# DearCaat/MHIM-MIL

Measured on AMD Instinct MI355X. Metric: patch-instances/sec through MHIM fwd+bwd, N=10k D=1024, higher is better.
Workload: dtype f32; 1 GPU; c2: MHIM(ABMIL) train step, one bag N=10000 D=1024 per GPU per step (teacher fwd + select + student fwd + bwd + Adam + EMA); rotating_bags_per_gpu=8, matrix_core_form=bf16x3, parallelism=dp1, launch=hipGraph replay, one graph per resident bag

## Files before the change

include/mhimx.h:

```cpp
#ifndef MHIMX_H
#define MHIMX_H

#include <stdint.h>

#ifdef __cplusplus
extern "C" {
#endif

#define MHIMX_VERSION 620

enum { MHIMX_ACT_NONE = 0, MHIMX_ACT_RELU = 1, MHIMX_ACT_GELU = 2, MHIMX_ACT_TANH = 3 };

enum { MHIMX_PREC_F32 = 0, MHIMX_PREC_F16S = 1, MHIMX_PREC_BF16X3 = 2 };

const char* mhimx_last_error(void);
int mhimx_version(void);


typedef struct {
  const float* A; int64_t lda; const int64_t* rows;
  const float* B; int64_t ldb;
  float* C; int64_t ldc;
  int64_t M, N, K;
  const float* bias;
// ... 257 lines not shown
  mhimx_reduce_list* defer;
} mhimx_merge_grad;
int64_t mhimx_merge_part_floats(void);
int mhimx_merge_fwd_part(void* stream, const mhimx_merge* m, const float* X, int64_t R, float* part, void* ws, int64_t ws_bytes);
int mhimx_merge_fwd_finish(void* stream, const mhimx_merge* m, const float* parts, int32_t W, int64_t R, float* z, float* q_new,
                           int32_t update_q, void* ws, int64_t ws_bytes);
int mhimx_merge_bwd(void* stream, const mhimx_merge* m, const float* X, int64_t R, const float* dz, float* dX,
                    const mhimx_merge_grad* g, void* ws, int64_t ws_bytes);
int mhimx_merge_bwd_park(const mhimx_merge* m, const float* X, int64_t R, const float* dz, float* dX, const mhimx_merge_grad* g, void* ws,
                         int64_t ws_bytes);

int mhimx_act_bwd(void* stream, float* dH, const float* H, const float* pre, int64_t M, int64_t E, int32_t act,
                  float drop_p, uint64_t drop_seed, const uint8_t* drop_mask, const int64_t* rows, float* colsum_out,
                  int32_t accumulate, void* ws, int64_t ws_bytes, const uint64_t* drop_tick);
int mhimx_mul_colsum(void* stream, float* dH, const float* dact, int64_t M, int64_t E, float* colsum_out, int32_t accumulate,
                     void* ws, int64_t ws_bytes, mhimx_reduce_list* defer );
int mhimx_rows_dpre(void* stream, const float* dH, const void* dact16, const int64_t* rows, int64_t L, int64_t E, float* dpre,
                    float* colsum_out, int32_t accumulate, void* ws, int64_t ws_bytes, mhimx_reduce_list* defer );
int64_t mhimx_wgrad_image_bytes(int64_t L, int64_t E);
int mhimx_rows_dpre_image(void* stream, const float* dH, const void* dact16, const int64_t* rows, int64_t L, int64_t E, void* img,
                          float* colsum_out, int32_t accumulate, void* ws, int64_t ws_bytes, mhimx_reduce_list* defer );
int mhimx_rows_dpre_image_c(void* stream, const float* dH_compact, const void* dact16, const int64_t* rows, int64_t L, int64_t E, void* img,
                            float* colsum_out, int32_t accumulate, void* ws, int64_t ws_bytes, mhimx_reduce_list* defer );
int mhimx_rows_dpre_image_k(void* stream, const float* dH, const void* dact16, const uint8_t* keep, int64_t N, int64_t E, void* img,
                            float* colsum_out, int32_t accumulate, void* ws, int64_t ws_bytes, mhimx_reduce_list* defer );
typedef struct {
  const void* img;
  const float* X; int64_t ldx; int64_t n_bag_rows;
  const int64_t* rows;
  int64_t L, E, D;
  float* C; int64_t ldc; int32_t accumulate;
  float* ws; int64_t ws_floats;
  mhimx_reduce_list* defer;
  int32_t ride_tail;
  const void* ximg;
} mhimx_bag_wgrad_args;
int64_t mhimx_wgrad_ws_floats(int64_t L, int64_t E, int64_t D);
int mhimx_bag_wgrad(void* stream, const mhimx_bag_wgrad_args* a);
int64_t mhimx_wgrad_multi_ws_floats(int64_t L, int64_t E, int64_t D, int32_t n_bags);
int mhimx_bag_wgrad_multi(void* stream, const mhimx_bag_wgrad_args* bags, int32_t n_bags);
int mhimx_shard_flags(void* stream, const int64_t* rows_all, int64_t R, int64_t Lk, int64_t lo, int64_t n, int64_t k_tokens,
                      int32_t tokens_live, uint8_t* excl);
int mhimx_shard_gather(void* stream, const float* H, int64_t E, const int64_t* rows, int64_t R, int64_t lo, int64_t n, float* out);
int mhimx_shard_scatter(void* stream, const float* dX, int64_t E, const int64_t* rows, int64_t R, int64_t lo, int64_t n, float* dH);
int mhimx_colsum(void* stream, const float* X, int64_t M, int64_t E, float* out, int32_t accumulate,
                 void* ws, int64_t ws_bytes);

int mhimx_head_fwd_bwd(void* stream, const float* z, const float* t, const float* wp, const float* bp,
                       const int64_t* label_dev, int64_t E, int64_t C, float temp_t, float main_alpha,
                       float aux_alpha, float inv_accum, float* logits, float* losses, float* g_z, float* d_wp,
                       float* d_bp, int32_t accumulate, const float* g_logits_in, const float* g_cl_in);

int mhimx_softmax_cols(void* stream, const float* x, float* y, int64_t M, int64_t C, float alpha);
int mhimx_softmax_cols_bwd(void* stream, const float* y, const float* dy, float* dx, int64_t M, int64_t C, float alpha);
int mhimx_colmax(void* stream, const float* x, int64_t M, int64_t C, float* vals, int64_t* idx);
int mhimx_rowmax(void* stream, const float* x, int64_t M, int64_t C, float* out);
int mhimx_dsmil_head(void* stream, const float* logits_bag, const float* logits_ins, const int64_t* label_dev, const float* Bs,
                     const float* Bt, int64_t C, int64_t V, float temp_t, float main_alpha, float aux_alpha, float inv_accum,
                     float* losses, float* g_logits_bag, float* g_logits_ins, float* g_B, const float* g_cl_in);

int mhimx_adam_ema(void* stream, float* p, const float* g, float* m, float* v, float* teacher, int64_t n_train,
                   int64_t n_all, int64_t step, float lr, float beta1, float beta2, float eps, float weight_decay,
                   float grad_scale, float ema_mm, int32_t zero_grad ,
                   const uint64_t* step_dev ,
                   const float* mm_table, int64_t mm_len );

typedef struct {
  float* p; float* g; float* m; float* v; float* teacher;
  int64_t n_train, n_all;
  int64_t step; const uint64_t* step_dev;
  float lr; const float* lr_table; int64_t lr_len;
  float beta1, beta2, eps, weight_decay, grad_scale;
  float ema_mm; const float* mm_table; int64_t mm_len;
  int32_t zero_grad;
  const float* g_extra; int64_t n_extra; int64_t extra_pitch;
  float clip_norm;
  float* ws; int64_t ws_floats;
  mhimx_reduce_list* fold;
  int64_t extra_lo;
  int32_t extra_only;
} mhimx_optim_args;
int mhimx_optim_step(void* stream, const mhimx_optim_args* a);

#define MHIMX_STEP_MAX_ROWS 262144
#define MHIMX_WINDOW_MAX 8
typedef struct {
  const float* w1; const float* b1;
  const float* wa; const float* wc;
  const float* wp; const float* bp;
  float* q;
  const float* ln_w; const float* ln_b;
  const float* wkv; const float* wq; const float* wo; const float* bo;
} mhimx_step_params;
typedef struct {
  float* w1; float* b1; float* wa; float* wc; float* wp; float* bp; float* ln_w; float* ln_b; float* wkv; float* wq; float* wo; float* bo;
} mhimx_step_grads;
typedef struct {
  int64_t D, E, A, C, k;
  int32_t act, da_act;
  int32_t attn2score;
  float drop_p_teacher, drop_p_student;
  float merge_drop_p, merge_mm;
  float temp_t, main_alpha, aux_alpha;
  mhimx_step_params student, teacher;
  mhimx_step_grads grad;
  float* p; float* g; float* m; float* v; float* p_teacher;
  int64_t n_train, n_all;
  float lr, beta1, beta2, eps, weight_decay, ema_mm;
  const float* mm_table; int64_t mm_len; const float* lr_table; int64_t lr_len;
  uint64_t* tick; uint64_t* opt_step;
  float* q_out;
  int32_t time_project;
  void* side_stream;
} mhimx_step_cfg;
typedef struct { int64_t k_top, n_sel, len_keep, Lk, R; } mhimx_step_counts;
int mhimx_step_counts_of(int64_t N, double mask_ratio_h, double mask_ratio_hr, double merge_ratio, mhimx_step_counts* out);
typedef struct { uint64_t drop_teacher, drop_student, select, mca; } mhimx_step_seeds;
typedef struct {
  int64_t total;
  int64_t logits, losses;
  int64_t score;
  int64_t rows_all;
  int64_t H_teacher, H_student;
  int64_t dact;
  int64_t z_teacher, z_student, g_z;
  int64_t dH;
} mhimx_step_layout;
int mhimx_step_layout_of(const mhimx_step_cfg* cfg, int64_t N, const mhimx_step_counts* cnt, mhimx_step_layout* out);
int mhimx_step_run(void* stream, const mhimx_step_cfg* cfg, const float* X, int64_t ldx, int64_t N, const int64_t* label_dev,
                   const mhimx_step_counts* cnt, const mhimx_step_seeds* seeds, int64_t host_step, void* ws, int64_t ws_bytes, int32_t update);
int mhimx_step_project_ms(float* ms_out, float* empty_ms_out, int32_t cap);
int mhimx_step_run_many(void* stream, const mhimx_step_cfg* cfg, int32_t n_bags, const float* const* X, const int64_t* ldx, const int64_t* N,
                        const int64_t* const* labels_dev, const mhimx_step_counts* cnt, const mhimx_step_seeds* seeds, int64_t host_step0,
                        void* ws, int64_t ws_bytes);

int mhimx_pure_step_layout_of(const mhimx_step_cfg* cfg, int64_t N, mhimx_step_layout* out);
int mhimx_pure_step_run(void* stream, const mhimx_step_cfg* cfg, const float* X, int64_t ldx, int64_t N, const int64_t* label_dev,
                        uint64_t drop_seed, int64_t host_step, void* ws, int64_t ws_bytes, int32_t update);
int mhimx_pure_step_run_many(void* stream, const mhimx_step_cfg* cfg, int32_t n_bags, const float* const* X, const int64_t* ldx, const int64_t* N,
                             const int64_t* const* labels_dev, const uint64_t* drop_seeds, int64_t host_step0, void* ws, int64_t ws_bytes);

typedef struct { int64_t total, bag0, bag_stride, grad_slab; mhimx_step_layout bag; } mhimx_window_layout;
int mhimx_window_layout_of(const mhimx_step_cfg* cfg, int32_t n_bags, int64_t N, const mhimx_step_counts* cnt, mhimx_window_layout* out);
int mhimx_window_run(void* stream, const mhimx_step_cfg* cfg, int32_t n_bags, const float* const* X, int64_t ldx, int64_t N,
                     const int64_t* const* labels_dev, const mhimx_step_counts* cnt, const mhimx_step_seeds* seeds, int64_t host_step, void* ws,
                     int64_t ws_bytes, int32_t update);

#define MHIMX_PURE_WINDOW_MAX 32
#define MHIMX_PURE_WINDOW_MAX_ROWS 524288
typedef struct {
  const float* X; int64_t ldx, N;
  const int64_t* label_dev;
  uint64_t drop_seed;
} mhimx_pure_window_bag;
typedef struct {
  int64_t total, rows;
  int64_t logits, losses;
  int64_t H, dact, s, stats, z, g_z;
  int64_t row0[MHIMX_PURE_WINDOW_MAX];
} mhimx_pure_window_layout;
int mhimx_pure_window_layout_of(const mhimx_step_cfg* cfg, int32_t n_bags, const mhimx_pure_window_bag* bags, mhimx_pure_window_layout* out);
int mhimx_pure_window_run(void* stream, const mhimx_step_cfg* cfg, int32_t n_bags, const mhimx_pure_window_bag* bags, int64_t host_step,
                          void* ws, int64_t ws_bytes, int32_t update);

#define MHIMX_RAGGED_WINDOW_MAX 32
#define MHIMX_RAGGED_WINDOW_MAX_ROWS 524288
typedef struct {
  const float* X; int64_t ldx, N;
  const int64_t* label_dev;
  mhimx_step_counts cnt;
  mhimx_step_seeds seeds;
} mhimx_ragged_window_bag;
typedef struct {
  int64_t total, rows;
  int64_t logits, losses;
  int64_t score;
  int64_t rows_all;
  int64_t H_teacher, H_student;
  int64_t dact;
  int64_t dpre;
  int64_t z_teacher, z_student;
  int64_t row0[MHIMX_RAGGED_WINDOW_MAX];
} mhimx_ragged_window_layout;
int mhimx_ragged_window_layout_of(const mhimx_step_cfg* cfg, int32_t n_bags, const mhimx_ragged_window_bag* bags,
                                  mhimx_ragged_window_layout* out);
int mhimx_ragged_window_run(void* stream, const mhimx_step_cfg* cfg, int32_t n_bags, const mhimx_ragged_window_bag* bags, int64_t host_step,
                            void* ws, int64_t ws_bytes, int32_t update);

#define MHIMX_INFER_MAX 32
#define MHIMX_INFER_MAX_ROWS 4194304
typedef struct {
  int64_t D, E, A, C;
  int32_t act, da_act;
  mhimx_step_params p;
} mhimx_infer_cfg;
typedef struct {
  const float* X; int64_t ldx;
  int64_t N;
} mhimx_infer_bag;
typedef struct {
  float* logits;
  float* z;
  float* stats;
  float* score;
  float* attn;
  float* loss;
} mhimx_infer_out;
int64_t mhimx_infer_ws_bytes(const mhimx_infer_cfg* cfg, int32_t n_bags, const mhimx_infer_bag* bags);
int mhimx_infer_run(void* stream, const mhimx_infer_cfg* cfg, int32_t n_bags, const mhimx_infer_bag* bags, const int64_t* labels_dev,
                    const mhimx_infer_out* out, void* ws, int64_t ws_bytes);

#define MHIMX_X_F32 0
#define MHIMX_X_F16 1
#define MHIMX_X_BF16 2
int mhimx_infer_run_x(void* stream, const mhimx_infer_cfg* cfg, int32_t n_bags, const mhimx_infer_bag* bags, const int64_t* labels_dev,
                      const mhimx_infer_out* out, void* ws, int64_t ws_bytes, int32_t x_dtype);
int mhimx_pure_window_run_x(void* stream, const mhimx_step_cfg* cfg, int32_t n_bags, const mhimx_pure_window_bag* bags, int64_t host_step,
// ... 23 lines not shown
```

mhim_mil_amd/_lib.py:

```python
from __future__ import annotations

import ctypes as C
import os

HERE = os.path.dirname(os.path.abspath(__file__))
LIB_PATH = os.path.join(HERE, os.environ.get("MHIMX_LIB_NAME", "libmhimx.so"))

c_f32p = C.c_void_p
c_i64p = C.c_void_p
c_u8p = C.c_void_p

ABI_VERSION = 620

ACT = {None: 0, "none": 0, "identity": 0, "relu": 1, "gelu": 2, "tanh": 3}
PREC = {"f32": 0, "f16s": 1, "bf16x3": 2}


def act_code(name, allowed):
    n = name.lower() if isinstance(name, str) else None
    return ACT[n] if n in allowed else 0


class GemmNT(C.Structure):
    _fields_ = [("A", c_f32p), ("lda", C.c_int64), ("rows", c_i64p),
# ... 58 lines not shown


class ReduceListC(C.Structure):
    _fields_ = [("j", ReduceJob * REDUCE_MAX), ("n", C.c_int32), ("side", SideWork), ("parked", ParkedGemm), ("pre", SideWork)]


class GemmTN(C.Structure):
    _fields_ = [("A", c_f32p), ("lda", C.c_int64),
                ("B", c_f32p), ("ldb", C.c_int64), ("rows", c_i64p),
                ("C", c_f32p), ("ldc", C.c_int64),
                ("M", C.c_int64), ("K1", C.c_int64), ("K2", C.c_int64),
                ("splits", C.c_int32), ("ws", c_f32p),
                ("accumulate", C.c_int32), ("prec", C.c_int32), ("ws_floats", C.c_int64),
                ("defer", C.c_void_p)]


class Scorer(C.Structure):
    _fields_ = [("E", C.c_int64), ("A", C.c_int64), ("act", C.c_int32), ("gated", C.c_int32), ("prec", C.c_int32),
                ("wa", c_f32p), ("ba", c_f32p), ("wb", c_f32p), ("bb", c_f32p), ("wc", c_f32p), ("bc", c_f32p),
                ("wa_frag", c_f32p), ("gate_drop_p", C.c_float), ("gate_drop_seed", C.c_uint64)]


class PoolIO(C.Structure):
    _fields_ = [("T1", c_f32p), ("M1", C.c_int64), ("T2", c_f32p), ("M2", C.c_int64),
                ("s", c_f32p), ("stats", c_f32p), ("z", c_f32p), ("u_pre", c_f32p),
                ("wp", c_f32p), ("C", C.c_int64), ("cproj", c_f32p),
                ("ws", C.c_void_p), ("ws_bytes", C.c_int64), ("bp", c_f32p), ("pscore", c_f32p), ("rows1", c_i64p),
                ("excl", C.c_void_p), ("ride_jobs", C.c_void_p), ("n_ride_jobs", C.c_int32),
                ("phase", C.c_int32), ("tail_tokens", C.c_int32), ("ride_merge", C.c_void_p), ("ride_X", c_f32p), ("ride_R", C.c_int64),
                ("ride_ws", C.c_void_p), ("ride_ws_bytes", C.c_int64), ("rode_merge", C.c_int32), ("tail_wa_t", c_f32p), ("tail_row0", C.c_int64),
                ("no_backward", C.c_int32)]


class PoolGrad(C.Structure):
    _fields_ = [("g_z", c_f32p), ("dT1", c_f32p), ("dT2", c_f32p),
                ("d_wa", c_f32p), ("d_ba", c_f32p), ("d_wb", c_f32p), ("d_bb", c_f32p), ("d_wc", c_f32p),
                ("d_bc", c_f32p), ("wa_t", c_f32p), ("wb_t", c_f32p),
                ("accumulate", C.c_int32), ("splits", C.c_int32), ("defer", C.c_void_p), ("wa_t_frag", c_f32p),
                ("img", C.c_void_p), ("img_dact", C.c_void_p), ("img_part", c_f32p), ("img_rows", C.c_int64)]


class Merge(C.Structure):
    _fields_ = [("E", C.c_int64), ("k", C.c_int64), ("heads", C.c_int64), ("dim_head", C.c_int64),
                ("q_param", c_f32p), ("ln_w", c_f32p), ("ln_b", c_f32p),
                ("wkv", c_f32p), ("wq", c_f32p), ("wo", c_f32p), ("bo", c_f32p),
                ("wkv_t", c_f32p), ("wq_t", c_f32p), ("wo_t", c_f32p),
                ("mm", C.c_float), ("drop_p", C.c_float), ("drop_seed", C.c_uint64), ("prec", C.c_int32), ("drop_tick", C.c_void_p),
                ("wkv_frag", c_f32p), ("x_rows", c_i64p), ("prepared", C.c_int32), ("own_lo", C.c_int64), ("own_n", C.c_int64),
                ("rep", C.c_float), ("rows_done", C.c_int32)]


class MergeGrad(C.Structure):
    _fields_ = [("d_ln_w", c_f32p), ("d_ln_b", c_f32p), ("d_wkv", c_f32p), ("d_wq", c_f32p), ("d_wo", c_f32p),
                ("d_bo", c_f32p), ("accumulate", C.c_int32), ("splits", C.c_int32), ("defer", C.c_void_p)]


_P = C.c_void_p
_I64 = C.c_int64
_I32 = C.c_int32
_F = C.c_float
_U64 = C.c_uint64


class Nys(C.Structure):
    _fields_ = [("q", C.c_void_p), ("k", C.c_void_p), ("v", C.c_void_p), ("ld", C.c_int64), ("T", C.c_int64),
                ("ql", C.c_void_p), ("kl", C.c_void_p), ("ldl", C.c_int64), ("scale", C.c_float),
                ("ws", C.c_void_p), ("ws_floats", C.c_int64)]


class BmmStep(C.Structure):
    _fields_ = [("A", C.c_void_p), ("B", C.c_void_p), ("C", C.c_void_p), ("PN", C.c_void_p), ("PT", C.c_void_p),
                ("PN2", C.c_void_p), ("PT2", C.c_void_p), ("D", C.c_void_p), ("D2", C.c_void_p), ("alpha", C.c_float), ("ident", C.c_float),
                ("alpha2", C.c_float), ("ident2", C.c_float), ("dscale", C.c_float), ("d2scale", C.c_float), ("kind", C.c_int32)]


class OptimArgs(C.Structure):
    _fields_ = [("p", C.c_void_p), ("g", C.c_void_p), ("m", C.c_void_p), ("v", C.c_void_p), ("teacher", C.c_void_p),
                ("n_train", C.c_int64), ("n_all", C.c_int64), ("step", C.c_int64), ("step_dev", C.c_void_p),
                ("lr", C.c_float), ("lr_table", C.c_void_p), ("lr_len", C.c_int64),
                ("beta1", C.c_float), ("beta2", C.c_float), ("eps", C.c_float), ("weight_decay", C.c_float), ("grad_scale", C.c_float),
                ("ema_mm", C.c_float), ("mm_table", C.c_void_p), ("mm_len", C.c_int64), ("zero_grad", C.c_int32),
                ("g_extra", C.c_void_p), ("n_extra", C.c_int64), ("extra_pitch", C.c_int64), ("clip_norm", C.c_float),
                ("ws", C.c_void_p), ("ws_floats", C.c_int64), ("fold", C.c_void_p), ("extra_lo", C.c_int64), ("extra_only", C.c_int32)]


class StepParams(C.Structure):
    _fields_ = [(n, C.c_void_p) for n in ("w1", "b1", "wa", "wc", "wp", "bp", "q", "ln_w", "ln_b", "wkv", "wq", "wo", "bo")]


class StepGrads(C.Structure):
    _fields_ = [(n, C.c_void_p) for n in ("w1", "b1", "wa", "wc", "wp", "bp", "ln_w", "ln_b", "wkv", "wq", "wo", "bo")]


class StepCfg(C.Structure):
    _fields_ = [("D", C.c_int64), ("E", C.c_int64), ("A", C.c_int64), ("C", C.c_int64), ("k", C.c_int64),
                ("act", C.c_int32), ("da_act", C.c_int32), ("attn2score", C.c_int32),
                ("drop_p_teacher", C.c_float), ("drop_p_student", C.c_float), ("merge_drop_p", C.c_float), ("merge_mm", C.c_float),
                ("temp_t", C.c_float), ("main_alpha", C.c_float), ("aux_alpha", C.c_float),
                ("student", StepParams), ("teacher", StepParams), ("grad", StepGrads),
                ("p", C.c_void_p), ("g", C.c_void_p), ("m", C.c_void_p), ("v", C.c_void_p), ("p_teacher", C.c_void_p),
                ("n_train", C.c_int64), ("n_all", C.c_int64),
                ("lr", C.c_float), ("beta1", C.c_float), ("beta2", C.c_float), ("eps", C.c_float), ("weight_decay", C.c_float), ("ema_mm", C.c_float),
                ("mm_table", C.c_void_p), ("mm_len", C.c_int64), ("lr_table", C.c_void_p), ("lr_len", C.c_int64),
                ("tick", C.c_void_p), ("opt_step", C.c_void_p), ("q_out", C.c_void_p), ("time_project", C.c_int32), ("side_stream", C.c_void_p)]


class StepCounts(C.Structure):
    _fields_ = [("k_top", C.c_int64), ("n_sel", C.c_int64), ("len_keep", C.c_int64), ("Lk", C.c_int64), ("R", C.c_int64)]


class StepSeeds(C.Structure):
    _fields_ = [("drop_teacher", C.c_uint64), ("drop_student", C.c_uint64), ("select", C.c_uint64), ("mca", C.c_uint64)]


class StepLayout(C.Structure):
    _fields_ = [(n, C.c_int64) for n in ("total", "logits", "losses", "score", "rows_all", "H_teacher", "H_student", "dact", "z_teacher",
                                        "z_student", "g_z", "dH")]


class WindowLayout(C.Structure):
    _fields_ = [("total", C.c_int64), ("bag0", C.c_int64), ("bag_stride", C.c_int64), ("grad_slab", C.c_int64), ("bag", StepLayout)]


WINDOW_MAX = 8
STEP_MAX_ROWS = 262144


class InferCfg(C.Structure):
    _fields_ = [("D", C.c_int64), ("E", C.c_int64), ("A", C.c_int64), ("C", C.c_int64), ("act", C.c_int32), ("da_act", C.c_int32),
                ("p", StepParams)]


class InferBag(C.Structure):
    _fields_ = [("X", c_f32p), ("ldx", C.c_int64), ("N", C.c_int64)]


class InferOut(C.Structure):
    _fields_ = [(n, c_f32p) for n in ("logits", "z", "stats", "score", "attn", "loss")]


INFER_MAX = 32
INFER_MAX_ROWS = 4194304
X_F32, X_F16, X_BF16 = 0, 1, 2

PURE_WINDOW_MAX = 32
PURE_WINDOW_MAX_ROWS = 524288


class PureWindowBag(C.Structure):
    _fields_ = [("X", c_f32p), ("ldx", C.c_int64), ("N", C.c_int64), ("label_dev", C.c_void_p), ("drop_seed", C.c_uint64)]


class PureWindowLayout(C.Structure):
    _fields_ = [(n, C.c_int64) for n in ("total", "rows", "logits", "losses", "H", "dact", "s", "stats", "z", "g_z")] + [
        ("row0", C.c_int64 * PURE_WINDOW_MAX)]


RAGGED_WINDOW_MAX = 32
RAGGED_WINDOW_MAX_ROWS = 524288


class RaggedWindowBag(C.Structure):
    _fields_ = [("X", c_f32p), ("ldx", C.c_int64), ("N", C.c_int64), ("label_dev", C.c_void_p), ("cnt", StepCounts), ("seeds", StepSeeds)]


class RaggedWindowLayout(C.Structure):
    _fields_ = [(n, C.c_int64) for n in ("total", "rows", "logits", "losses", "score", "rows_all", "H_teacher", "H_student", "dact", "dpre",
                                        "z_teacher", "z_student")] + [("row0", C.c_int64 * RAGGED_WINDOW_MAX)]


SYMBOLS = {
    "mhimx_last_error": (C.c_char_p, []),
    "mhimx_version": (C.c_int, []),
    "mhimx_gemm_nt": (C.c_int, [_P, C.POINTER(GemmNT)]),
    "mhimx_pool_finalize": (C.c_int, [_P, _P, _P, _P, _I64, _I64, _P, _P, _P, _P, _P, _I64, _I64, _P]),
    "mhimx_proj_score_parts": (_I64, [_I64]),
    "mhimx_proj_score_xch_floats": (_I64, [_I64]),
    "mhimx_bag_project": (C.c_int, [_P, C.POINTER(BagProject)]),
    "mhimx_bag_project_multi": (C.c_int, [_P, _P, _I32]),
    "mhimx_gemm_nn": (C.c_int, [_P, C.POINTER(GemmNT), _F, _I32, _P]),
    "mhimx_prep_batch": (C.c_int, [_P, C.POINTER(PrepJob), _I32]),
    "mhimx_pair_planes": (C.c_int, [_P, _P, _I64, _I64, _I64, _P]),
    "mhimx_lse_merge": (C.c_int, [_P, _P, _I64, _I64, _P, _P]),
    "mhimx_gemm_batched": (C.c_int, [_P, _I32, C.POINTER(GemmNT), _I32, _I64, _I64, _I64, _F, _I32, _P]),
    "mhimx_gemm_tn": (C.c_int, [_P, C.POINTER(GemmTN)]),
    "mhimx_transpose": (C.c_int, [_P, _P, _P, _I64, _I64]),
    "mhimx_abmil_pool_ws_bytes": (_I64, [_I64, _I64, _I64, _I32]),
    "mhimx_abmil_pool_fwd": (C.c_int, [_P, C.POINTER(Scorer), C.POINTER(PoolIO)]),
    "mhimx_abmil_pool_bwd": (C.c_int, [_P, C.POINTER(Scorer), C.POINTER(PoolIO), C.POINTER(PoolGrad)]),
    "mhimx_softmax_from_stats": (C.c_int, [_P, _P, _P, _P, _I64]),
    "mhimx_pseudo_score": (C.c_int, [_P, _P, _P, _P, _P, _P, _P, _I64, _I64]),
    "mhimx_select_ws_bytes": (_I64, [_I64]),
    "mhimx_select_mask": (C.c_int, [_P, _P, _I64, _I64, _I64, _I32, _P, _P, _I64, _P, _P, _P, _P, _I64]),
    "mhimx_select_rows": (C.c_int, [_P, _P, _I64, _I64, _I64, _I32, _U64, _P, _I64, _P, _P, _P, _I64, _I32]),
    "mhimx_select_rows_img": (C.c_int, [_P, _P, _I64, _I64, _I64, _I32, _U64, _P, _I64, _P, _P, _I64, _P, _I64, _I32]),
    "mhimx_vote_scores": (C.c_int, [_P, _P, _I64, _I64, _I64, _I32, _P, _P, _I64]),
    "mhimx_compose_ids": (C.c_int, [_P, _P, _P, _P, _I64]),
    "mhimx_random_perm": (C.c_int, [_P, _I64, _U64, _P, _P, _P]),
    "mhimx_merge_ws_bytes": (_I64, [_I64, _I64, _I64, _I64, _I64]),
    "mhimx_merge_fwd": (C.c_int, [_P, C.POINTER(Merge), _P, _I64, _P, _P, _I32, _P, _I64]),
    "mhimx_merge_part_floats": (_I64, []),
    "mhimx_merge_fwd_part": (C.c_int, [_P, C.POINTER(Merge), _P, _I64, _P, _P, _I64]),
    "mhimx_merge_fwd_finish": (C.c_int, [_P, C.POINTER(Merge), _P, _I32, _I64, _P, _P, _I32, _P, _I64]),
    "mhimx_merge_bwd": (C.c_int, [_P, C.POINTER(Merge), _P, _I64, _P, _P, C.POINTER(MergeGrad), _P, _I64]),
    "mhimx_merge_bwd_park": (C.c_int, [C.POINTER(Merge), _P, _I64, _P, _P, C.POINTER(MergeGrad), _P, _I64]),
    "mhimx_act_bwd": (C.c_int, [_P, _P, _P, _P, _I64, _I64, _I32, _F, _U64, _P, _P, _P, _I32, _P, _I64, _P]),
    "mhimx_softmax_cols": (C.c_int, [_P, _P, _P, _I64, _I64, _F]),
    "mhimx_softmax_cols_bwd": (C.c_int, [_P, _P, _P, _P, _I64, _I64, _F]),
    "mhimx_colmax": (C.c_int, [_P, _P, _I64, _I64, _P, _P]),
    "mhimx_rowmax": (C.c_int, [_P, _P, _I64, _I64, _P]),
    "mhimx_dsmil_head": (C.c_int, [_P, _P, _P, _P, _P, _P, _I64, _I64, _F, _F, _F, _F, _P, _P, _P, _P, _P]),
    "mhimx_mul_colsum": (C.c_int, [_P, _P, _P, _I64, _I64, _P, _I32, _P, _I64, _P]),
    "mhimx_rows_dpre": (C.c_int, [_P, _P, _P, _P, _I64, _I64, _P, _P, _I32, _P, _I64, _P]),
    "mhimx_bmm_affine": (C.c_int, [_P, _I32, _P, _I32, _I64, _I64, _I64, C.c_float, C.c_float]),
    "mhimx_bmm_affine2": (C.c_int, [_P, _I32, _P, _I32, _I64, _I64, _I64, C.c_float, C.c_float, _P, C.c_float, C.c_float]),
    "mhimx_bmm_affine_pair": (C.c_int, [_P, _I32, C.POINTER(GemmNT), _F, _F, _I32, C.POINTER(GemmNT), _F, _F, _I32, _I64]),
    "mhimx_shard_flags": (C.c_int, [_P, _P, _I64, _I64, _I64, _I64, _I64, _I32, _P]),
    "mhimx_shard_gather": (C.c_int, [_P, _P, _I64, _P, _I64, _I64, _I64, _P]),
    "mhimx_shard_scatter": (C.c_int, [_P, _P, _I64, _P, _I64, _I64, _I64, _P]),
    "mhimx_rows_dpre_image": (C.c_int, [_P, _P, _P, _P, _I64, _I64, _P, _P, _I32, _P, _I64, _P]),
    "mhimx_rows_dpre_image_c": (C.c_int, [_P, _P, _P, _P, _I64, _I64, _P, _P, _I32, _P, _I64, _P]),
    "mhimx_rows_dpre_image_k": (C.c_int, [_P, _P, _P, _P, _I64, _I64, _P, _P, _I32, _P, _I64, _P]),
    "mhimx_wgrad_image_bytes": (_I64, [_I64, _I64]),
    "mhimx_wgrad_ws_floats": (_I64, [_I64, _I64, _I64]),
    "mhimx_bag_wgrad": (C.c_int, [_P, _P]),
    "mhimx_bag_wgrad_multi": (C.c_int, [_P, _P, _I32]),
    "mhimx_wgrad_multi_ws_floats": (C.c_int64, [_I64, _I64, _I64, _I32]),
    "mhimx_reduce_flush": (C.c_int, [_P, _P]),
    "mhimx_cls_metrics_ws_bytes": (C.c_int64, [_I64, _I64, _I64]),
    "mhimx_cls_metrics": (C.c_int, [_P, _P, _I64, _P, _I64, _I64, _I32, _P, _I64, _P, _P, _I64]),
    "mhimx_colsum": (C.c_int, [_P, _P, _I64, _I64, _P, _I32, _P, _I64]),
    "mhimx_head_fwd_bwd": (C.c_int, [_P, _P, _P, _P, _P, _P, _I64, _I64, _F, _F, _F, _F, _P, _P, _P, _P, _P, _I32, _P, _P]),
    "mhimx_adam_ema": (C.c_int, [_P, _P, _P, _P, _P, _P, _I64, _I64, _I64, _F, _F, _F, _F, _F, _F, _F, _I32, _P, _P, _I64]),
    "mhimx_bmm_chain": (C.c_int, [_P, C.POINTER(BmmStep), _I32, _I32, _P]),
    "mhimx_optim_step": (C.c_int, [_P, C.POINTER(OptimArgs)]),
    "mhimx_stream_copy": (C.c_int, [_P, _P, _P, _I64]),
    "mhimx_tick": (C.c_int, [_P, _P]),
    "mhimx_layernorm_fwd": (C.c_int, [_P, _P, _I64, _I64, _P, _P, _P, _P, _P]),
    "mhimx_layernorm_bwd": (C.c_int, [_P, _P, _P, _I64, _I64, _P, _P, _P, _P, _P, _P, _I32, _P]),
    "mhimx_layernorm_bwd_res": (C.c_int, [_P, _P, _P, _I64, _I64, _P, _P, _P, _P, _P, _P, _P, _I32, _P]),
    "mhimx_dropout_apply": (C.c_int, [_P, _P, _P, _I64, _I64, _F, _U64, _P]),
    "mhimx_dropout_apply_proj": (C.c_int, [_P, _P, _P, _I64, _I64, _F, _U64, _P]),
    "mhimx_softmax_rows": (C.c_int, [_P, _P, _P, _I64, _I64, _F]),
    "mhimx_softmax_rows_bwd": (C.c_int, [_P, _P, _P, _P, _I64, _I64, _F]),
    "mhimx_landmark_mean": (C.c_int, [_P, _P, _I64, _I64, _I64, _I64, _P]),
    "mhimx_landmark_mean_bwd": (C.c_int, [_P, _P, _I64, _I64, _I64, _P, _I64, _I32]),
    "mhimx_affine_ident": (C.c_int, [_P, _P, _P, _I64, _I64, _F, _F]),
    "mhimx_axpby": (C.c_int, [_P, _P, _P, _I64, _F, _F]),
    "mhimx_pinv_init": (C.c_int, [_P, _P, _I64, _I64, _P, _P, _P]),
    "mhimx_pinv_init_bwd": (C.c_int, [_P, _P, _P, _P, _I64, _I64, _P, _P]),
    "mhimx_comm_unique_id": (C.c_int, [_P]),
    "mhimx_comm_init": (C.c_int, [C.POINTER(C.c_void_p), _P, _I32, _I32]),
    "mhimx_comm_allreduce": (C.c_int, [_P, _P, _P, _I64, _I32]),
    "mhimx_comm_destroy": (C.c_int, [_P]),
    "mhimx_bn_ws_floats": (_I64, [_I64, _I64]),
    "mhimx_bn_fwd": (C.c_int, [_P, _P, _I64, _I64, _P, _P, C.c_float, _I32, _P, _P, _P, _P, _P]),
    "mhimx_bn_bwd": (C.c_int, [_P, _P, _P, _I64, _I64, _P, _P, _P, _I32, _P, _P, _P, _P]),
    "mhimx_sincos_add": (C.c_int, [_P, _P, _P, _I64, _I64, _P]),
    "mhimx_nys_ws_floats": (_I64, [_I64]),
    "mhimx_nys_a3v_fwd": (C.c_int, [_P, C.POINTER(Nys), _P, _P]),
    "mhimx_nys_out_fwd": (C.c_int, [_P, C.POINTER(Nys), _P, _P, _I64, _P, C.c_int32]),
    "mhimx_nys_out_bwd": (C.c_int, [_P, C.POINTER(Nys), _P, _P, _I64, _P, _P, _P, _I64, _P, _I64, _P]),
    "mhimx_nys_a3v_bwd": (C.c_int, [_P, C.POINTER(Nys), _P, _P, _P, _P, _P, _I64, _I32, _P, _I64]),
    "mhimx_nys_cls_attn": (C.c_int, [_P, C.POINTER(Nys), _P, _P, _P]),
    "mhimx_resconv": (C.c_int, [_P, _P, _I64, _P, _I64, _I64, _I64, _I64, _P, _I64, _I32, _I32]),
    "mhimx_resconv_dw_ws_floats": (_I64, [_I64, _I64, _I64, _I64]),
    "mhimx_resconv_dw": (C.c_int, [_P, _P, _I64, _P, _I64, _I64, _I64, _I64, _I64, _P, _P]),
    "mhimx_ppeg_combine": (C.c_int, [_P, _P, _P, _P, _P, _P, _P, _I64, _P, _P]),
    "mhimx_ppeg_fwd": (C.c_int, [_P, _P, _I64, _I64, _P, _P, _P, _I64]),
    "mhimx_ppeg_bwd_ws_floats": (_I64, [_I64, _I64]),
    "mhimx_ppeg_bwd": (C.c_int, [_P, _P, _P, _I64, _I64, _P, _P, _P, _P, _P, _I64]),
    "mhimx_ppeg_side": (_I64, [_I64, _P]),
    "mhimx_ppeg_band_fwd": (C.c_int, [_P, _P, _P, _I64, _P, _P, _P]),
    "mhimx_ppeg_band_bwd_ws_floats": (_I64, [_I64, _I64]),
    "mhimx_ppeg_band_bwd": (C.c_int, [_P, _P, _P, _P, _I64, _I64, _P, _P, _P, _P, _P]),
    "mhimx_scale_heads": (C.c_int, [_P, _P, _I64, _P, _I64, _I64, _I64, _I64, _P]),
    "mhimx_step_counts_of": (C.c_int, [_I64, C.c_double, C.c_double, C.c_double, C.POINTER(StepCounts)]),
    "mhimx_step_layout_of": (C.c_int, [C.POINTER(StepCfg), _I64, C.POINTER(StepCounts), C.POINTER(StepLayout)]),
    "mhimx_step_run": (C.c_int, [_P, C.POINTER(StepCfg), _P, _I64, _I64, _P, C.POINTER(StepCounts), C.POINTER(StepSeeds), _I64, _P, _I64, _I32]),
    "mhimx_step_project_ms": (C.c_int, [_P, _P, _I32]),
    "mhimx_window_layout_of": (C.c_int, [C.POINTER(StepCfg), _I32, _I64, C.POINTER(StepCounts), C.POINTER(WindowLayout)]),
    "mhimx_window_run": (C.c_int, [_P, C.POINTER(StepCfg), _I32, _P, _I64, _I64, _P, C.POINTER(StepCounts), C.POINTER(StepSeeds), _I64, _P, _I64, _I32]),
    "mhimx_infer_ws_bytes": (_I64, [C.POINTER(InferCfg), _I32, _P]),
    "mhimx_infer_run": (C.c_int, [_P, C.POINTER(InferCfg), _I32, _P, _P, C.POINTER(InferOut), _P, _I64]),
    "mhimx_infer_run_x": (C.c_int, [_P, C.POINTER(InferCfg), _I32, _P, _P, C.POINTER(InferOut), _P, _I64, _I32]),
    "mhimx_step_run_many": (C.c_int, [_P, C.POINTER(StepCfg), _I32, _P, _P, _P, _P, C.POINTER(StepCounts), C.POINTER(StepSeeds), _I64, _P, _I64]),
    "mhimx_pure_step_layout_of": (C.c_int, [C.POINTER(StepCfg), _I64, C.POINTER(StepLayout)]),
    "mhimx_pure_step_run": (C.c_int, [_P, C.POINTER(StepCfg), _P, _I64, _I64, _P, C.c_uint64, _I64, _P, _I64, _I32]),
    "mhimx_pure_step_run_many": (C.c_int, [_P, C.POINTER(StepCfg), _I32, _P, _P, _P, _P, _P, _I64, _P, _I64]),
    "mhimx_pure_window_layout_of": (C.c_int, [C.POINTER(StepCfg), _I32, _P, C.POINTER(PureWindowLayout)]),
    "mhimx_pure_window_run": (C.c_int, [_P, C.POINTER(StepCfg), _I32, _P, _I64, _P, _I64, _I32]),
    "mhimx_pure_window_run_x": (C.c_int, [_P, C.POINTER(StepCfg), _I32, _P, _I64, _P, _I64, _I32, _I32]),
    "mhimx_ragged_window_layout_of": (C.c_int, [C.POINTER(StepCfg), _I32, _P, C.POINTER(RaggedWindowLayout)]),
    "mhimx_ragged_window_run": (C.c_int, [_P, C.POINTER(StepCfg), _I32, _P, _I64, _P, _I64, _I32]),
    "mhimx_ragged_window_run_x": (C.c_int, [_P, C.POINTER(StepCfg), _I32, _P, _I64, _P, _I64, _I32, _I32]),
}

_lib = None


def lib():
    global _lib
    if _lib is not None:
        return _lib
    if not os.path.exists(LIB_PATH):
        raise RuntimeError(
            f"{LIB_PATH} not found: the MI355X HIP library has not been built "
            f"(run `python -m mhim_mil_amd.build` or __graft_entry__.build()); there is no fallback path")
    import torch
    L = C.CDLL(LIB_PATH)
    for name, (res, args) in SYMBOLS.items():
        fn = getattr(L, name)
        fn.restype = res
        fn.argtypes = args
    if L.mhimx_version() != ABI_VERSION:
        raise RuntimeError(f"{LIB_PATH} is ABI version {L.mhimx_version()}, this binding expects {ABI_VERSION}: a stale build "
                           f"(rebuild with `python -m mhim_mil_amd.build --force`)")
    _lib = L
    return L


class MhimxError(RuntimeError):
    pass


def check(status: int, what: str = ""):
    if status != 0:
        msg = lib().mhimx_last_error()
        raise MhimxError(f"{what} failed with status {status}: {msg.decode() if msg else ''}")
```

mhim_mil_amd/csrc/optim.hip:

```cpp
#include <math.h>

#include "common.hpp"

namespace mhimx {

int reduce_flush(hipStream_t st, mhimx_reduce_list* list);

constexpr int HEAD_THREADS = 256;

MHIMX_DEV float blk_sum(float v, float* red) {
  v = wave_sum(v);
  __syncthreads();
  if ((threadIdx.x & 63) == 0) red[threadIdx.x >> 6] = v;
  __syncthreads();
  return red[0] + red[1] + red[2] + red[3];
}
MHIMX_DEV float blk_max(float v, float* red) {
  v = wave_max(v);
  __syncthreads();
  if ((threadIdx.x & 63) == 0) red[threadIdx.x >> 6] = v;
  __syncthreads();
  return fmaxf(fmaxf(red[0], red[1]), fmaxf(red[2], red[3]));
}

// ... 230 lines not shown
      g_lb[tid] = g;
      g_li[tid] = g;
    }
  }
  if (g_cl_in) aux_alpha = g_cl_in[0];
  float cl = 0.f;
  if (Bt) {
    for (int c = 0; c < C; ++c) {
      const float* s = Bs + (int64_t)c * V;
      const float* t = Bt + (int64_t)c * V;
      float a = -INFINITY, b = -INFINITY;
      for (int e = tid; e < V; e += HEAD_THREADS) { a = fmaxf(a, s[e]); b = fmaxf(b, t[e] / temp_t); }
      const float smx = blk_max(a, red), tmx = blk_max(b, red);
      float sa = 0.f, sb = 0.f;
      for (int e = tid; e < V; e += HEAD_THREADS) { sa += expf(s[e] - smx); sb += expf(t[e] / temp_t - tmx); }
      const float sden = blk_sum(sa, red), tden = blk_sum(sb, red);
      const float ls = logf(sden);
      float acc = 0.f;
      for (int e = tid; e < V; e += HEAD_THREADS) {
        const float pt = expf(t[e] / temp_t - tmx) / tden;
        acc += pt * (s[e] - smx - ls);
        if (g_B) g_B[(int64_t)c * V + e] = aux_alpha * inv_accum / (float)C * (expf(s[e] - smx) / sden - pt);
      }
      cl -= blk_sum(acc, red) / (float)C;
    }
  } else if (g_B) {
    for (int i = tid; i < C * V; i += HEAD_THREADS) g_B[i] = 0.f;
  }
  if (tid == 0) {
    losses[0] = main_alpha * ce + aux_alpha * cl;
    losses[1] = ce;
    losses[2] = cl;
  }
}

constexpr int FOLD_MAX = 4;
struct FoldJobs { const float* parts[FOLD_MAX]; int64_t off[FOLD_MAX], n[FOLD_MAX]; int G[FOLD_MAX], accumulate[FOLD_MAX]; int count; };
struct OptimExtra { const float* lr_table; int64_t lr_len; const float* g_extra; int64_t n_extra, extra_pitch; float clip_norm;
                    const float* sq_parts; int n_parts; FoldJobs fold; int64_t extra_lo; int extra_only; };

MHIMX_DEV float4 fold_sum4(const float* __restrict__ parts, int64_t n, int64_t idx, int G) {
  float4 s0 = make_float4(0.f, 0.f, 0.f, 0.f), s1 = s0, s2 = s0, s3 = s0;
  auto ld = [&](int z) { return *reinterpret_cast<const float4*>(parts + (int64_t)z * n + idx); };
  auto add = [](float4& a, const float4& b) { a.x += b.x; a.y += b.y; a.z += b.z; a.w += b.w; };
  int z = 0;
  for (; z + 8 <= G; z += 8) {
    const float4 p0 = ld(z), p1 = ld(z + 1), p2 = ld(z + 2), p3 = ld(z + 3), p4 = ld(z + 4), p5 = ld(z + 5), p6 = ld(z + 6), p7 = ld(z + 7);
    add(s0, p0); add(s1, p1); add(s2, p2); add(s3, p3);
    add(s0, p4); add(s1, p5); add(s2, p6); add(s3, p7);
  }
  for (; z + 4 <= G; z += 4) { add(s0, ld(z)); add(s1, ld(z + 1)); add(s2, ld(z + 2)); add(s3, ld(z + 3)); }
  for (; z < G; ++z) add(s0, ld(z));
  return make_float4((s0.x + s1.x) + (s2.x + s3.x), (s0.y + s1.y) + (s2.y + s3.y), (s0.z + s1.z) + (s2.z + s3.z), (s0.w + s1.w) + (s2.w + s3.w));
}

__global__ __launch_bounds__(256) void grad_sumsq_kernel(const float* __restrict__ g, int64_t n, float gscale, OptimExtra ex, float* __restrict__ parts) {
  __shared__ float red[256];
  float a = 0.f;
  for (int64_t i = (int64_t)blockIdx.x * 256 + threadIdx.x; i < n; i += (int64_t)gridDim.x * 256) {
    const bool slabs = i >= ex.extra_lo;
    float v = (slabs && ex.extra_only) ? 0.f : g[i];
    if (slabs)
      for (int64_t z = 0; z < ex.n_extra; ++z) v += ex.g_extra[z * ex.extra_pitch + i];
    v *= gscale;
    a += v * v;
  }
  red[threadIdx.x] = a;
  __syncthreads();
  for (int o = 128; o > 0; o >>= 1) {
    if ((int)threadIdx.x < o) red[threadIdx.x] += red[threadIdx.x + o];
    __syncthreads();
  }
  if (threadIdx.x == 0) parts[blockIdx.x] = red[0];
}

MHIMX_DEV void adam_one(float& w, float& gi, float& mi, float& vi, float lr_over_bc1, float bc2s, float beta1, float beta2,
                        float eps, float wd, float gscale) {
  gi = gi * gscale + wd * w;
  mi = beta1 * mi + (1.f - beta1) * gi;
  vi = beta2 * vi + (1.f - beta2) * gi * gi;
  w = w - lr_over_bc1 * (mi / (sqrtf(vi) / bc2s + eps));
}

__global__ __launch_bounds__(256) void adam_ema_kernel(
    float* __restrict__ p, float* __restrict__ g, float* __restrict__ m, float* __restrict__ v, float* __restrict__ teacher,
    int64_t n_train, int64_t n_all, float lr_over_bc1, float bc2s, float beta1, float beta2, float eps, float wd, float gscale,
    float mm, int zero_grad, const uint64_t* __restrict__ step_dev, float lr, const float* __restrict__ mm_table, int64_t mm_len,
    int64_t step_host, double ln_beta1, double ln_beta2, OptimExtra ex) {
  __shared__ float sc[4];
  __shared__ float clip_red[256];
  if (ex.clip_norm > 0.f) {
    float a = 0.f;
    for (int i = threadIdx.x; i < ex.n_parts; i += 256) a += ex.sq_parts[i];
    clip_red[threadIdx.x] = a;
    __syncthreads();
    for (int o = 128; o > 0; o >>= 1) {
      if ((int)threadIdx.x < o) clip_red[threadIdx.x] += clip_red[threadIdx.x + o];
      __syncthreads();
    }
  }
  if (threadIdx.x == 0) {
    int64_t step = step_host;
    if (step_dev) step = (int64_t)step_dev[0];
    if (ex.lr_table) {
      int64_t i = step - 1;
      i = i < 0 ? 0 : (i >= ex.lr_len ? ex.lr_len - 1 : i);
      lr = ex.lr_table[i];
    }
    if (step_dev || ex.lr_table) {
      const double t = (double)step;
      lr_over_bc1 = (float)((double)lr / (1.0 - exp(t * ln_beta1)));
      bc2s = (float)sqrt(1.0 - exp(t * ln_beta2));
    }
    float coef = 1.f;
    if (ex.clip_norm > 0.f) {
      coef = ex.clip_norm / (sqrtf(clip_red[0]) + 1e-6f);
      coef = coef > 1.f ? 1.f : coef;
    }
    sc[3] = coef;
    if (mm_table) {
      int64_t i = step - 1;
      i = i < 0 ? 0 : (i >= mm_len ? mm_len - 1 : i);
      mm = mm_table[i];
    }
    sc[0] = lr_over_bc1; sc[1] = bc2s; sc[2] = mm;
  }
  __syncthreads();
  lr_over_bc1 = sc[0];
  bc2s = sc[1];
  mm = sc[2];
  gscale *= sc[3];
  const int64_t n4 = n_all / 4;
  const bool vec_ok = ((reinterpret_cast<uintptr_t>(p) | reinterpret_cast<uintptr_t>(g) | reinterpret_cast<uintptr_t>(m) |
                        reinterpret_cast<uintptr_t>(v) | reinterpret_cast<uintptr_t>(teacher)) & 15) == 0;
  for (int64_t q = (int64_t)blockIdx.x * blockDim.x + threadIdx.x; q * 4 < n_all; q += (int64_t)gridDim.x * blockDim.x) {
    const int64_t i0 = q * 4;
    if (vec_ok && q < n4 && (i0 + 4 <= n_train || i0 >= n_train)) {
      float4 w = reinterpret_cast<float4*>(p)[q];
      if (i0 < n_train) {
        const bool slabs = i0 >= ex.extra_lo;
        float4 gi = (slabs && ex.extra_only) ? make_float4(0.f, 0.f, 0.f, 0.f) : reinterpret_cast<float4*>(g)[q];
        float4 mi = reinterpret_cast<float4*>(m)[q], vi = reinterpret_cast<float4*>(v)[q];
        for (int f = 0; f < ex.fold.count; ++f)
          if (i0 >= ex.fold.off[f] && i0 < ex.fold.off[f] + ex.fold.n[f]) {
            const float4 sv = fold_sum4(ex.fold.parts[f], ex.fold.n[f], i0 - ex.fold.off[f], ex.fold.G[f]);
            if (ex.fold.accumulate[f]) { gi.x += sv.x; gi.y += sv.y; gi.z += sv.z; gi.w += sv.w; }
            else gi = sv;
          }
        for (int64_t z = 0; slabs && z < ex.n_extra; ++z) {
          const float4 e = *reinterpret_cast<const float4*>(ex.g_extra + z * ex.extra_pitch + i0);
          gi.x += e.x; gi.y += e.y; gi.z += e.z; gi.w += e.w;
        }
        adam_one(w.x, gi.x, mi.x, vi.x, lr_over_bc1, bc2s, beta1, beta2, eps, wd, gscale);
        adam_one(w.y, gi.y, mi.y, vi.y, lr_over_bc1, bc2s, beta1, beta2, eps, wd, gscale);
        adam_one(w.z, gi.z, mi.z, vi.z, lr_over_bc1, bc2s, beta1, beta2, eps, wd, gscale);
        adam_one(w.w, gi.w, mi.w, vi.w, lr_over_bc1, bc2s, beta1, beta2, eps, wd, gscale);
        reinterpret_cast<float4*>(m)[q] = mi;
        reinterpret_cast<float4*>(v)[q] = vi;
        reinterpret_cast<float4*>(p)[q] = w;
        if (zero_grad) reinterpret_cast<float4*>(g)[q] = make_float4(0.f, 0.f, 0.f, 0.f);
      }
      if (teacher) {
        float4 t = reinterpret_cast<float4*>(teacher)[q];
        t.x = t.x * mm + w.x * (1.f - mm); t.y = t.y * mm + w.y * (1.f - mm);
        t.z = t.z * mm + w.z * (1.f - mm); t.w = t.w * mm + w.w * (1.f - mm);
        reinterpret_cast<float4*>(teacher)[q] = t;
      }
      continue;
    }
    for (int64_t i = i0; i < i0 + 4 && i < n_all; ++i) {
      float w = p[i];
      if (i < n_train) {
        const bool slabs = i >= ex.extra_lo;
        float gi = (slabs && ex.extra_only) ? 0.f : g[i], mi = m[i], vi = v[i];
        for (int64_t z = 0; slabs && z < ex.n_extra; ++z) gi += ex.g_extra[z * ex.extra_pitch + i];
        adam_one(w, gi, mi, vi, lr_over_bc1, bc2s, beta1, beta2, eps, wd, gscale);
        m[i] = mi;
        v[i] = vi;
        p[i] = w;
        if (zero_grad) g[i] = 0.f;
      }
      if (teacher) teacher[i] = teacher[i] * mm + w * (1.f - mm);
    }
  }
}

}

using namespace mhimx;

extern "C" int mhimx_head_fwd_bwd(void* stream, const float* z, const float* t, const float* wp, const float* bp,
                                  const int64_t* label_dev, int64_t E, int64_t C, float temp_t, float main_alpha,
                                  float aux_alpha, float inv_accum, float* logits, float* losses, float* g_z, float* d_wp,
                                  float* d_bp, int32_t accumulate, const float* g_logits_in, const float* g_cl_in) {
  MHIMX_CHECK_ARG(z && wp && logits && losses && g_z, "head: null args");
  MHIMX_CHECK_ARG(C > 0 && C <= 16 && E > 0, "head: bad dims");
  if (C <= 4 && E <= 2 * HEAD_THREADS)
    hipLaunchKernelGGL(head_fast_kernel<2>, bgrid(1), dim3(HEAD_THREADS), 0, (hipStream_t)stream, z, t, wp, bp, label_dev, (int)E, (int)C,
                     temp_t, main_alpha, aux_alpha, inv_accum, logits, losses, g_z, d_wp, d_bp, accumulate, g_logits_in, g_cl_in, cur_batch());
  else if (C <= 4 && E <= 4 * HEAD_THREADS)
    hipLaunchKernelGGL(head_fast_kernel<4>, bgrid(1), dim3(HEAD_THREADS), 0, (hipStream_t)stream, z, t, wp, bp, label_dev, (int)E, (int)C,
                     temp_t, main_alpha, aux_alpha, inv_accum, logits, losses, g_z, d_wp, d_bp, accumulate, g_logits_in, g_cl_in, cur_batch());
  else if (cur_batch().n > 0)
    return fail(-1, "head: a bag-batched launch takes the short-chain head (C <= 4, E <= 1024)");
  else
  hipLaunchKernelGGL(head_kernel, dim3(1), dim3(HEAD_THREADS), 0, (hipStream_t)stream, z, t, wp, bp, label_dev, (int)E, (int)C,
                     temp_t, main_alpha, aux_alpha, inv_accum, logits, losses, g_z, d_wp, d_bp, accumulate, g_logits_in, g_cl_in);
  MHIMX_LAUNCH_CHECK();
  return 0;
}

extern "C" int mhimx_dsmil_head(void* stream, const float* logits_bag, const float* logits_ins, const int64_t* label_dev,
                                const float* Bs, const float* Bt, int64_t C, int64_t V, float temp_t, float main_alpha,
                                float aux_alpha, float inv_accum, float* losses, float* g_logits_bag, float* g_logits_ins,
                                float* g_B, const float* g_cl_in) {
  MHIMX_CHECK_ARG(losses && Bs && C > 0 && C <= 16 && V > 0, "dsmil_head: bad args");
  MHIMX_CHECK_ARG(!label_dev || (logits_bag && logits_ins && g_logits_bag && g_logits_ins), "dsmil_head: label needs the logits and their gradients");
  hipLaunchKernelGGL(dsmil_head_kernel, dim3(1), dim3(HEAD_THREADS), 0, (hipStream_t)stream, logits_bag, logits_ins, label_dev, Bs, Bt,
                     (int)C, (int)V, temp_t, main_alpha, aux_alpha, inv_accum, losses, g_logits_bag, g_logits_ins, g_B, g_cl_in);
  MHIMX_LAUNCH_CHECK();
  return 0;
}

extern "C" int mhimx_optim_step(void* stream, const mhimx_optim_args* a) {
  MHIMX_CHECK_ARG(a, "optim_step: null args");
  MHIMX_CHECK_ARG(!a->mm_table || a->mm_len > 0, "optim_step: empty momentum schedule");
  MHIMX_CHECK_ARG(!a->lr_table || a->lr_len > 0, "optim_step: empty learning-rate schedule");
  MHIMX_CHECK_ARG(a->p && a->g && a->m && a->v && a->n_train >= 0 && a->n_all >= a->n_train && (a->step >= 1 || a->step_dev), "optim_step: bad args");
  MHIMX_CHECK_ARG(a->n_extra >= 0 && (a->n_extra == 0 || (a->g_extra && a->extra_pitch >= a->n_train && a->extra_pitch % 4 == 0 && aligned16(a->g_extra))),
                  "optim_step: gradient slabs need a 16-byte aligned base and a pitch >= n_train that is a multiple of 4");
  MHIMX_CHECK_ARG(!(a->clip_norm > 0.f) || (a->ws && a->ws_floats >= 1024), "optim_step: clipping needs a workspace of 1024 floats");
  MHIMX_CHECK_ARG(a->extra_lo >= 0 && a->extra_lo % 4 == 0 && (a->n_extra > 0 || (a->extra_lo == 0 && !a->extra_only)),
                  "optim_step: extra_lo (a multiple of 4) / extra_only describe the gradient slabs of g_extra");
  int64_t step = a->step < 1 ? 1 : a->step;
  if (a->n_all == 0) return 0;
  OptimExtra ex{a->lr_table, a->lr_len, a->g_extra, a->n_extra, a->extra_pitch, a->clip_norm > 0.f ? a->clip_norm : 0.f, a->ws, 0, {}, a->extra_lo, a->extra_only};
  if (a->fold) {
    mhimx_reduce_list* l = a->fold;
    MHIMX_CHECK_ARG(l->n >= 0 && l->n <= MHIMX_REDUCE_MAX, "optim_step: bad reduction list");
    const bool vec_ok = aligned16(a->p) && aligned16(a->g) && aligned16(a->m) && aligned16(a->v) && (!a->teacher || aligned16(a->teacher));
    if (!(a->clip_norm > 0.f) && vec_ok) {
      int kept = 0;
      for (int i = 0; i < l->n; ++i) {
        const mhimx_reduce_job& j = l->j[i];
        const int64_t n = j.K1 * j.K2, off = j.out - a->g;
        const bool take = j.kind == 1 && ex.fold.count < FOLD_MAX && j.G >= 1 && j.G <= 64 && j.ldo == j.K2 && n > 0 && n % 4 == 0 && aligned16(j.parts) &&
                          j.out >= a->g && off % 4 == 0 && off + n <= a->n_train / 4 * 4;
        if (take) {
          const int f = ex.fold.count++;
          ex.fold.parts[f] = j.parts; ex.fold.off[f] = off; ex.fold.n[f] = n; ex.fold.G[f] = (int)j.G; ex.fold.accumulate[f] = j.accumulate;
        } else {
          l->j[kept++] = j;
        }
      }
      l->n = kept;
    }
    if (l->n > 0 || l->side.pending || l->parked.pending)
      if (int r = reduce_flush((hipStream_t)stream, l)) return r;
  }
  if (ex.clip_norm > 0.f && a->n_train > 0) {
    const int64_t nb = cdiv(a->n_train, 1024) < 1024 ? cdiv(a->n_train, 1024) : 1024;
    ex.n_parts = (int)nb;
    hipLaunchKernelGGL(grad_sumsq_kernel, dim3((unsigned)nb), dim3(256), 0, (hipStream_t)stream, a->g, a->n_train, a->grad_scale, ex, a->ws);
    MHIMX_LAUNCH_CHECK();
  } else {
    ex.clip_norm = 0.f;
  }
  const double bc1 = 1.0 - pow((double)a->beta1, (double)step);
  const double bc2 = 1.0 - pow((double)a->beta2, (double)step);
  const int64_t blocks = cdiv(a->n_all, 1024) < 2048 ? cdiv(a->n_all, 1024) : 2048;
  hipLaunchKernelGGL(adam_ema_kernel, dim3((unsigned)blocks), dim3(256), 0, (hipStream_t)stream, a->p, a->g, a->m, a->v,
                     a->teacher, a->n_train, a->n_all, (float)((double)a->lr / bc1), (float)sqrt(bc2), a->beta1, a->beta2, a->eps, a->weight_decay,
                     a->grad_scale, a->ema_mm, a->zero_grad, a->step_dev, a->lr, a->mm_table, a->mm_len, step, log((double)a->beta1),
                     log((double)a->beta2), ex);
  MHIMX_LAUNCH_CHECK();
  return 0;
}

extern "C" int mhimx_adam_ema(void* stream, float* p, const float* g, float* m, float* v, float* teacher, int64_t n_train,
                              int64_t n_all, int64_t step, float lr, float beta1, float beta2, float eps, float weight_decay,
                              float grad_scale, float ema_mm, int32_t zero_grad, const uint64_t* step_dev,
                              const float* mm_table, int64_t mm_len) {
  mhimx_optim_args a{};
  a.p = p; a.g = const_cast<float*>(g); a.m = m; a.v = v; a.teacher = teacher; a.n_train = n_train; a.n_all = n_all; a.step = step;
  a.step_dev = step_dev; a.lr = lr; a.beta1 = beta1; a.beta2 = beta2; a.eps = eps; a.weight_decay = weight_decay; a.grad_scale = grad_scale;
  a.ema_mm = ema_mm; a.mm_table = mm_table; a.mm_len = mm_len; a.zero_grad = zero_grad;
  return mhimx_optim_step(stream, &a);
}

typedef float sc_f4 __attribute__((ext_vector_type(4)));
__global__ __launch_bounds__(256) void stream_copy_kernel(const sc_f4* __restrict__ src, sc_f4* __restrict__ dst, int64_t n4) {
  const int64_t stride = (int64_t)gridDim.x * 256;
  for (int64_t i = (int64_t)blockIdx.x * 256 + threadIdx.x; i < n4; i += stride) __builtin_nontemporal_store(__builtin_nontemporal_load(src + i), dst + i);
}
extern "C" int mhimx_stream_copy(void* stream, const float* src, float* dst, int64_t n_floats) {
  MHIMX_CHECK_ARG(src && dst && n_floats >= 0 && n_floats % 4 == 0 && aligned16(src) && aligned16(dst), "stream_copy: 16-byte aligned buffers, n % 4 == 0");
  if (n_floats == 0) return 0;
  const int64_t n4 = n_floats / 4;
  const int64_t blocks = cdiv(n4, 256) < (1 << 20) ? cdiv(n4, 256) : (1 << 20);
  hipLaunchKernelGGL(stream_copy_kernel, dim3((unsigned)blocks), dim3(256), 0, (hipStream_t)stream, reinterpret_cast<const sc_f4*>(src),
                     reinterpret_cast<sc_f4*>(dst), n4);
  MHIMX_LAUNCH_CHECK();
  return 0;
}

__global__ void tick_kernel(uint64_t* c) { c[0] += 1; }
extern "C" int mhimx_tick(void* stream, uint64_t* counter) {
  MHIMX_CHECK_ARG(counter, "tick: null counter");
  hipLaunchKernelGGL(tick_kernel, dim3(1), dim3(1), 0, (hipStream_t)stream, counter);
  MHIMX_LAUNCH_CHECK();
  return 0;
}
```

mhim_mil_amd/csrc/step.hip:

```cpp
#include <math.h>
#include <string.h>

#include "common.hpp"

namespace mhimx {

int64_t merge2_rows_tiles(int64_t R);

namespace {

struct DagEvents {
  hipEvent_t e[64][6];
  bool have[64] = {};
  int get(hipEvent_t** out) {
    int dev = 0;
    MHIMX_HIP(hipGetDevice(&dev));
    MHIMX_CHECK_ARG(dev >= 0 && dev < 64, "step: device index %d", dev);
    if (!have[dev]) {
      for (int i = 0; i < 6; ++i) MHIMX_HIP(hipEventCreateWithFlags(&e[dev][i], hipEventDisableTiming));
      have[dev] = true;
    }
    *out = e[dev];
    return 0;
  }
// ... 102 lines not shown
  b->merge_ws = cv.take_off(b->merge_ws_bytes);
  b->fuse_img = N <= 16384;
  b->P0 = b->fuse_img ? (n->Lk + k + 31) / 32 * 32 : 0;
  b->L_img = b->fuse_img ? b->P0 + n->R : n->len_keep;
  b->H_t = cv.take_off(N * E * F);
  b->Hbuf = cv.take_off((N + k) * E * F);
  b->dact = cv.take_off(N * E * 2);
  b->s_t = cv.take_off(N * F);
  b->stats_t = cv.take_off(2 * F);
  b->z_t = cv.take_off(E * F);
  b->cproj_t = cv.take_off(N * C * F);
  b->pscore = cv.take_off(N * F);
  b->attn = cv.take_off(N * F);
  b->pool_ws_t_bytes = mhimx_abmil_pool_ws_bytes(N, E, A, 0);
  b->pool_ws_t = cv.take_off(b->pool_ws_t_bytes);
  b->rows_all = cv.take_off((n->len_keep + k) * 8);
  b->sel_ws_bytes = mhimx_select_ws_bytes(N);
  b->sel_ws = cv.take_off(b->sel_ws_bytes);
  b->rows_img = b->fuse_img ? cv.take_off((b->L_img + 31) / 32 * 32 * 8) : 0;
  b->sel_perm = b->sel_ids = b->sel_rows = b->sel_lk = 0;
  if (N > 16384) {
    b->sel_perm = cv.take_off(n->k_top * 8);
    b->sel_ids = cv.take_off(N * 8);
    b->sel_rows = cv.take_off(n->len_keep * 8);
    b->sel_lk = cv.take_off(8);
  }
  const int64_t M = n->Lk + k;
  b->s_s = cv.take_off(M * F);
  b->stats_s = cv.take_off(2 * F);
  b->z_s = cv.take_off(E * F);
  b->pool_ws_s_bytes = mhimx_abmil_pool_ws_bytes(M, E, A, 0);
  b->pool_ws_s = cv.take_off(b->pool_ws_s_bytes);
  b->logits = cv.take_off(16 * F);
  b->losses = cv.take_off(4 * F);
  b->g_z = cv.take_off(E * F);
  b->dH = cv.take_off((N + k) * E * F);
  b->img = cv.take_off(mhimx_wgrad_image_bytes(b->L_img, E));
  b->ws_b_bytes = (b->fuse_img ? b->P0 / 32 + (n->R + 31) / 32 : (n->len_keep + 31) / 32) * E * F;
  b->ws_b = cv.take_off(b->ws_b_bytes);
  b->q_scr = b->gslab = 0;
  if (n_bags > 1) {
    b->q_scr = cv.take_off(k * E * F);
    b->gslab = cv.take_off(c->n_all * F);
  } else {
    b->wg_ws_floats = mhimx_wgrad_ws_floats(b->L_img, E, D);
    b->wg_ws = cv.take_off(b->wg_ws_floats * F);
  }
  b->bag_stride = cv.off - b->bag0;
  b->total = b->bag0 + (int64_t)n_bags * b->bag_stride;
}

}

int step_check_cfg(const mhimx_step_cfg* c, int64_t N, const mhimx_step_counts* n) { return check_cfg(c, N, n); }

}

using namespace mhimx;

extern "C" int mhimx_step_counts_of(int64_t N, double mask_ratio_h, double mask_ratio_hr, double merge_ratio, mhimx_step_counts* out) {
  MHIMX_CHECK_ARG(out && N >= 1 && mask_ratio_h > 0.0 && mask_ratio_hr > 0.0 && merge_ratio > 0.0, "step_counts: bad arguments");
  double eff = mask_ratio_h / mask_ratio_hr, rr = mask_ratio_hr;
  if (eff > 1.0) { rr = mask_ratio_h; eff = 1.0; }
  const int64_t k = (int64_t)ceil((double)N * eff);
  const int64_t n_sel = rr < 1.0 ? (int64_t)ceil((double)k * rr) : k;
  const int64_t len_keep = N - n_sel;
  const int64_t Lk = (int64_t)((double)len_keep * merge_ratio);
  *out = mhimx_step_counts{k, n_sel, len_keep, Lk, len_keep - Lk};
  MHIMX_CHECK_ARG(k >= 1 && n_sel >= 1 && len_keep >= 1 && Lk >= 1 && len_keep - Lk >= 1, "step_counts: the recipe leaves nothing to mask, keep or merge");
  return 0;
}

extern "C" int mhimx_step_layout_of(const mhimx_step_cfg* cfg, int64_t N, const mhimx_step_counts* cnt, mhimx_step_layout* out) {
  MHIMX_CHECK_ARG(out, "step_layout: null output");
  if (int r = check_cfg(cfg, N, cnt)) return r;
  StepBufs b;
  layout(cfg, N, cnt, &b);
  *out = mhimx_step_layout{b.total, b.logits, b.losses, cfg->attn2score ? b.pscore : b.attn, b.rows_all, b.H_t, b.Hbuf, b.dact, b.z_t, b.z_s, b.g_z, b.dH};
  return 0;
}

extern "C" int mhimx_step_run(void* stream, const mhimx_step_cfg* cfg, const float* X, int64_t ldx, int64_t N, const int64_t* label_dev,
                              const mhimx_step_counts* cnt, const mhimx_step_seeds* seeds, int64_t host_step, void* ws, int64_t ws_bytes, int32_t update) {
  if (int r = check_cfg(cfg, N, cnt)) return r;
  MHIMX_CHECK_ARG(X && label_dev && seeds && ws && ldx >= cfg->D && ldx % 4 == 0 && N * ldx * 4 < ((int64_t)1 << 32) && aligned16(X),
                  "step: null bag / label / seeds / workspace, or a row pitch the weight-gradient product does not take");
  MHIMX_CHECK_ARG(!update || (cfg->p && cfg->g && cfg->m && cfg->v && cfg->n_train > 0 && cfg->n_all >= cfg->n_train), "step: update needs the flat optimiser buffers");
  StepBufs b;
  layout(cfg, N, cnt, &b);
  MHIMX_CHECK_ARG(ws_bytes >= b.total && (reinterpret_cast<uintptr_t>(ws) & 255) == 0, "step: workspace too small (%lld < %lld) or not 256-byte aligned",
                  (long long)ws_bytes, (long long)b.total);
  const mhimx_step_cfg& c = *cfg;
  const mhimx_step_params &S = c.student, &T = c.teacher;
  const int64_t D = c.D, E = c.E, A = c.A, C = c.C, k = c.k, I = 512;
  const int64_t R = cnt->R, Lk = cnt->Lk, len_keep = cnt->len_keep;
  Carve cv(ws);
  float* w1p_t = cv.at<float>(b.w1p_t);
  float* wa_frag_t = cv.at<float>(b.wa_frag_t);
  float* w1p_s = cv.at<float>(b.w1p_s);
  float* wa_frag_s = cv.at<float>(b.wa_frag_s);
  float* wa_t = cv.at<float>(b.wa_t);
  float* wa_t_frag = cv.at<float>(b.wa_t_frag);
  float* wo_t = cv.at<float>(b.wo_t);
  float* q_old = cv.at<float>(b.q_old);
  void* merge_ws = cv.at<char>(b.merge_ws);
  float* H_t = cv.at<float>(b.H_t);
  float* Hbuf = cv.at<float>(b.Hbuf);
  void* dact = cv.at<char>(b.dact);
  int64_t* rows_all = cv.at<int64_t>(b.rows_all);
  float* dH = cv.at<float>(b.dH);
  const uint64_t* tick = c.tick;
  const hipStream_t main_st = (hipStream_t)stream, side_st = (hipStream_t)c.side_stream;
  const bool dag = c.side_stream != nullptr && c.side_stream != stream;
  hipEvent_t* ev = nullptr;
  if (dag)
    if (int r = g_dag_events.get(&ev)) return r;

  mhimx_merge mw_prep = {};
  mw_prep.E = E; mw_prep.k = k; mw_prep.heads = 8; mw_prep.dim_head = 64;
  mw_prep.q_param = S.q; mw_prep.ln_w = S.ln_w; mw_prep.ln_b = S.ln_b; mw_prep.wkv = S.wkv; mw_prep.wq = S.wq; mw_prep.wo = S.wo; mw_prep.bo = S.bo;
  mw_prep.mm = c.merge_mm; mw_prep.prec = MHIMX_PREC_BF16X3; mw_prep.drop_tick = tick; mw_prep.rep = 1.f;
  {
    mhimx_prep_job early[8];
    int n = 0;
    early[n++] = mhimx_prep_job{3, nullptr, reinterpret_cast<float*>(c.tick), 1, 1};
    if (c.opt_step) early[n++] = mhimx_prep_job{3, nullptr, reinterpret_cast<float*>(c.opt_step), 1, 1};
    early[n++] = mhimx_prep_job{1, T.w1, w1p_t, E, D};
    early[n++] = mhimx_prep_job{4, T.wa, wa_frag_t, A, E};
    early[n++] = mhimx_prep_job{1, S.w1, w1p_s, E, D};
    early[n++] = mhimx_prep_job{10, nullptr, reinterpret_cast<float*>(rows_all + len_keep), N, k};
    if (int r = mhimx_prep_batch(stream, early, n)) return r;
  }
  mhimx_prep_job late[6];
  late[0] = mhimx_prep_job{4, S.wa, wa_frag_s, A, E};
  late[1] = mhimx_prep_job{0, S.wa, wa_t, A, E};
  late[2] = mhimx_prep_job{5, S.wa, wa_t_frag, A, E};
  late[3] = mhimx_prep_job{0, S.wo, wo_t, E, I};
  late[4] = mhimx_prep_job{2, S.q, q_old, 1, k * E};
  late[5] = mhimx_prep_job{6, reinterpret_cast<const float*>(&mw_prep), static_cast<float*>(merge_ws), R, b.merge_ws_bytes};

  {
    mhimx_bag_project_args a = {};
    a.X = X; a.ldx = ldx; a.N = N; a.D = D; a.E = E; a.act = c.act; a.n_heads = 2; a.drop_tick = tick;
    a.head[0].wp = w1p_t; a.head[0].bias = T.b1; a.head[0].H = H_t; a.head[0].ldh = E; a.head[0].drop_p = c.drop_p_teacher; a.head[0].drop_seed = seeds->drop_teacher;
    a.head[1].wp = w1p_s; a.head[1].bias = S.b1; a.head[1].H = Hbuf; a.head[1].ldh = E; a.head[1].dact = dact; a.head[1].drop_p = c.drop_p_student;
    a.head[1].drop_seed = seeds->drop_student;
    hipEvent_t* tp = nullptr;
    int tp_dev = 0;
    if (c.time_project) {
      hipStreamCaptureStatus cs = hipStreamCaptureStatusNone;
      MHIMX_HIP(hipStreamIsCapturing(main_st, &cs));
      if (cs == hipStreamCaptureStatusNone)
        if (int r = g_proj_times.next(&tp_dev, &tp)) return r;
    }
    if (tp) MHIMX_HIP(hipEventRecord(tp[0], main_st));
    if (int r = mhimx_bag_project(stream, &a)) return r;
    if (tp) {
      MHIMX_HIP(hipEventRecord(tp[1], main_st));
      MHIMX_HIP(hipEventRecord(tp[2], main_st));
      ++g_proj_times.n[tp_dev];
    }
  }

  mhimx_scorer sc_t = {};
  sc_t.E = E; sc_t.A = A; sc_t.act = c.da_act; sc_t.prec = MHIMX_PREC_BF16X3; sc_t.wa = T.wa; sc_t.wc = T.wc; sc_t.wa_frag = wa_frag_t;
  const float* score = nullptr;
  {
    mhimx_pool_io io = {};
    io.T1 = H_t; io.M1 = N; io.s = cv.at<float>(b.s_t); io.stats = cv.at<float>(b.stats_t); io.z = cv.at<float>(b.z_t);
    io.ws = cv.at<char>(b.pool_ws_t); io.ws_bytes = b.pool_ws_t_bytes;
    if (c.attn2score) { io.wp = T.wp; io.C = C; io.cproj = cv.at<float>(b.cproj_t); io.bp = T.bp; io.pscore = cv.at<float>(b.pscore); }
    io.no_backward = 1;
    io.ride_jobs = late; io.n_ride_jobs = 6;
    if (int r = mhimx_abmil_pool_fwd(stream, &sc_t, &io)) return r;
    if (c.attn2score) score = io.pscore;
    else {
      if (int r = mhimx_softmax_from_stats(stream, io.s, io.stats, cv.at<float>(b.attn), N)) return r;
      score = cv.at<float>(b.attn);
    }
  }
  const float* z_t = cv.at<float>(b.z_t);

  if (N <= 16384) {
    if (b.fuse_img) {
      if (int r = mhimx_select_rows_img(stream, score, N, cnt->k_top, cnt->n_sel, 1, seeds->select, tick, R, rows_all, cv.at<int64_t>(b.rows_img), b.P0,
                                        cv.at<char>(b.sel_ws), b.sel_ws_bytes, 1))
        return r;
    } else if (int r = mhimx_select_rows(stream, score, N, cnt->k_top, cnt->n_sel, 1, seeds->select, tick, R, rows_all, nullptr, cv.at<char>(b.sel_ws),
                                         b.sel_ws_bytes, 1))
      return r;
  } else {
    int64_t* perm = cv.at<int64_t>(b.sel_perm);
    int64_t* ids = cv.at<int64_t>(b.sel_ids);
    int64_t* rows = cv.at<int64_t>(b.sel_rows);
    if (int r = mhimx_random_perm(stream, cnt->k_top, seeds->select + 0x51ED270Bull, tick, nullptr, perm)) return r;
    if (int r = mhimx_select_mask(stream, score, N, cnt->k_top, cnt->n_sel, 1, cnt->n_sel < cnt->k_top ? perm : nullptr, nullptr, 0, ids, cv.at<int64_t>(b.sel_lk),
                                  nullptr, cv.at<char>(b.sel_ws), b.sel_ws_bytes))
      return r;
    if (int r = mhimx_random_perm(stream, len_keep, seeds->select ^ 0x3C6EF372FE94F82Bull, tick, ids, rows)) return r;
    MHIMX_HIP(hipMemcpyAsync(rows_all, rows + Lk, (size_t)R * 8, hipMemcpyDeviceToDevice, (hipStream_t)stream));
    MHIMX_HIP(hipMemcpyAsync(rows_all + R, rows, (size_t)Lk * 8, hipMemcpyDeviceToDevice, (hipStream_t)stream));
  }

  mhimx_merge mw = mw_prep;
  mw.drop_p = c.merge_drop_p; mw.drop_seed = seeds->mca; mw.x_rows = rows_all; mw.prepared = 1;
  mhimx_scorer sc_s = sc_t;
  sc_s.wa = S.wa; sc_s.wc = S.wc; sc_s.wa_frag = wa_frag_s;
  mhimx_pool_io io_s = {};
  io_s.T1 = Hbuf; io_s.M1 = Lk + k; io_s.s = cv.at<float>(b.s_s); io_s.stats = cv.at<float>(b.stats_s); io_s.z = cv.at<float>(b.z_s);
  io_s.ws = cv.at<char>(b.pool_ws_s); io_s.ws_bytes = b.pool_ws_s_bytes; io_s.rows1 = rows_all + R;
  io_s.tail_row0 = -1;
  if (dag && k <= 6) {
    if (int r = dag_edge(ev[0], main_st, side_st)) return r;
    io_s.phase = 1; io_s.tail_tokens = (int32_t)k;
    if (int r = mhimx_abmil_pool_fwd(side_st, &sc_s, &io_s)) return r;
    if (int r = mhimx_merge_fwd(stream, &mw, Hbuf, R, Hbuf + N * E, c.q_out ? c.q_out : S.q, 1, merge_ws, b.merge_ws_bytes)) return r;
    if (int r = dag_edge(ev[1], side_st, main_st)) return r;
    io_s.phase = 2; io_s.tail_wa_t = wa_t; io_s.tail_row0 = N;
    if (int r = mhimx_abmil_pool_fwd(stream, &sc_s, &io_s)) return r;
    io_s.phase = 0;
  } else if (k <= 6) {
    io_s.phase = 1; io_s.tail_tokens = (int32_t)k;
    io_s.ride_merge = &mw; io_s.ride_X = Hbuf; io_s.ride_R = R; io_s.ride_ws = merge_ws; io_s.ride_ws_bytes = b.merge_ws_bytes;
    if (int r = mhimx_abmil_pool_fwd(stream, &sc_s, &io_s)) return r;
    mw.rows_done = io_s.rode_merge;
    if (int r = mhimx_merge_fwd(stream, &mw, Hbuf, R, Hbuf + N * E, c.q_out ? c.q_out : S.q, 1, merge_ws, b.merge_ws_bytes)) return r;
    mw.rows_done = 0;
    io_s.phase = 2; io_s.tail_wa_t = wa_t; io_s.tail_row0 = N;
    if (int r = mhimx_abmil_pool_fwd(stream, &sc_s, &io_s)) return r;
    io_s.phase = 0; io_s.ride_merge = nullptr;
  } else {
    if (int r = mhimx_merge_fwd(stream, &mw, Hbuf, R, Hbuf + N * E, c.q_out ? c.q_out : S.q, 1, merge_ws, b.merge_ws_bytes)) return r;
    if (int r = mhimx_abmil_pool_fwd(stream, &sc_s, &io_s)) return r;
  }

  float* g_z = cv.at<float>(b.g_z);
  if (int r = mhimx_head_fwd_bwd(stream, io_s.z, c.aux_alpha != 0.f ? z_t : nullptr, S.wp, S.bp, label_dev, E, C, c.temp_t, c.main_alpha, c.aux_alpha, 1.f,
                                 cv.at<float>(b.logits), cv.at<float>(b.losses), g_z, c.grad.wp, c.grad.bp, 0, nullptr, nullptr))
    return r;

  mhimx_reduce_list lst;
  memset(&lst, 0, sizeof(lst));
  mhimx_merge mwb = mw;
  mwb.q_param = q_old; mwb.wo_t = wo_t; mwb.prepared = 0;
  mhimx_merge_grad mg = {};
  mg.d_ln_w = c.grad.ln_w; mg.d_ln_b = c.grad.ln_b; mg.d_wkv = c.grad.wkv; mg.d_wq = c.grad.wq; mg.d_wo = c.grad.wo; mg.d_bo = c.grad.bo;
  mg.accumulate = 0; mg.splits = 8; mg.defer = &lst;
  if (int r = mhimx_merge_bwd_park(&mwb, Hbuf, R, dH + N * E, dH, &mg, merge_ws, b.merge_ws_bytes)) return r;
  {
    mhimx_scorer sc_b = sc_s;
    sc_b.wa_frag = nullptr;
    mhimx_pool_grad pg = {};
    pg.g_z = g_z; pg.dT1 = dH; pg.d_wa = c.grad.wa; pg.d_wc = c.grad.wc; pg.wa_t = wa_t; pg.accumulate = 0; pg.splits = 8; pg.defer = &lst; pg.wa_t_frag = wa_t_frag;
    if (b.fuse_img) { pg.img = cv.at<char>(b.img); pg.img_dact = dact; pg.img_part = cv.at<float>(b.ws_b); pg.img_rows = Lk; }
    if (int r = mhimx_abmil_pool_bwd(stream, &sc_b, &io_s, &pg)) return r;
  }
  mhimx_reduce_list lst_main;
  memset(&lst_main, 0, sizeof(lst_main));
  mhimx_reduce_list* lm = dag ? &lst_main : &lst;
  if (dag) {
    if (int r = dag_edge(ev[2], main_st, side_st)) return r;
    if (lst.parked.pending && lst.pre.pending == 2) lst.parked.reserved = (int32_t)merge2_rows_tiles(R) + 1;
    if (int r = mhimx_reduce_flush(side_st, &lst)) return r;
  }
  if (int r = mhimx_merge_bwd(stream, &mwb, Hbuf, R, dH + N * E, dH, &mg, merge_ws, b.merge_ws_bytes)) return r;
  if (dag) {
    if (int r = dag_edge(ev[3], main_st, side_st)) return r;
    if (int r = mhimx_reduce_flush(side_st, &lst)) return r;
  }
  if (b.fuse_img) {
    if (int r = dpre_merge_rows(stream, dH, dact, rows_all, R, E, cv.at<char>(b.img), b.P0, c.grad.b1, cv.at<float>(b.ws_b), b.ws_b_bytes, lm)) return r;
  } else if (int r = mhimx_rows_dpre_image(stream, dH, dact, rows_all, len_keep, E, cv.at<char>(b.img), c.grad.b1, 0, cv.at<char>(b.ws_b), b.ws_b_bytes, lm))
    return r;
  {
    mhimx_bag_wgrad_args g = {};
    g.img = cv.at<char>(b.img); g.X = X; g.ldx = ldx; g.n_bag_rows = N; g.rows = b.fuse_img ? cv.at<int64_t>(b.rows_img) : rows_all; g.L = b.L_img; g.E = E; g.D = D;
    g.C = c.grad.w1; g.ldc = D;
    g.accumulate = 0; g.ws = cv.at<float>(b.wg_ws); g.ws_floats = b.wg_ws_floats; g.defer = lm; g.ride_tail = update ? 1 : 0;
    if (int r = mhimx_bag_wgrad(stream, &g)) return r;
  }
  if (dag)
    if (int r = dag_edge(ev[4], side_st, main_st)) return r;
  if (!update) return mhimx_reduce_flush(stream, lm);

  mhimx_optim_args o = {};
  o.p = c.p; o.g = c.g; o.m = c.m; o.v = c.v; o.teacher = c.p_teacher; o.n_train = c.n_train; o.n_all = c.n_all; o.step = host_step; o.step_dev = c.opt_step;
  o.lr = c.lr; o.lr_table = c.lr_table; o.lr_len = c.lr_len; o.beta1 = c.beta1; o.beta2 = c.beta2; o.eps = c.eps; o.weight_decay = c.weight_decay;
  o.grad_scale = 1.f; o.ema_mm = c.ema_mm; o.mm_table = c.mm_table; o.mm_len = c.mm_len; o.zero_grad = 1; o.fold = lm;
  return mhimx_optim_step(stream, &o);
}

namespace mhimx {
namespace {

struct QChainW { float wq; float w[MHIMX_WINDOW_MAX]; };
struct SlabGaps { int n; int64_t off[16], len[16]; };
__global__ __launch_bounds__(256) void window_q_chain_kernel(float* __restrict__ q, const float* __restrict__ z0, int64_t z_stride, int n_bags, int64_t n,
                                                             QChainW cw, float* __restrict__ slab0, int64_t pitch, SlabGaps gaps) {
  for (int64_t i = (int64_t)blockIdx.x * blockDim.x + threadIdx.x; i < n; i += (int64_t)gridDim.x * blockDim.x) {
    float acc = 0.f;
    for (int b = 0; b < n_bags; ++b) acc += z0[b * z_stride + i] * cw.w[b];
    q[i] = q[i] * cw.wq + acc;
  }
  for (int gi = 0; gi < gaps.n; ++gi)
    for (int b = 0; b < n_bags; ++b)
      for (int64_t i = (int64_t)blockIdx.x * blockDim.x + threadIdx.x; i < gaps.len[gi]; i += (int64_t)gridDim.x * blockDim.x)
        slab0[b * pitch + gaps.off[gi] + i] = 0.f;
}
__global__ __launch_bounds__(256) void window_sum_slabs_kernel(float* __restrict__ g, const float* __restrict__ slab0, int64_t pitch, int n_bags, int64_t n) {
  for (int64_t i = (int64_t)blockIdx.x * blockDim.x + threadIdx.x; i < n; i += (int64_t)gridDim.x * blockDim.x) {
    float acc = 0.f;
    for (int b = 0; b < n_bags; ++b) acc += slab0[b * pitch + i];
    g[i] = acc;
  }
}

int check_window(const mhimx_step_cfg* c, int32_t n_bags, int64_t N, const mhimx_step_counts* n) {
  if (int r = check_cfg(c, N, n)) return r;
  MHIMX_CHECK_ARG(n_bags >= 2 && n_bags <= MHIMX_WINDOW_MAX, "window: 2..%d bags", MHIMX_WINDOW_MAX);
  MHIMX_CHECK_ARG(N <= 16384 && c->k <= 6, "window: bags of up to 16384 rows (the one-workgroup select), merge_k <= 6");
  MHIMX_CHECK_ARG(c->g && c->n_train > 0 && c->n_all >= c->n_train && c->n_all % 4 == 0, "window: the flat gradient buffer (n_all %% 4 == 0) is required");
  MHIMX_CHECK_ARG(!c->q_out && !c->side_stream, "window: q_out / side_stream are single-step options");
  const mhimx_step_grads& g = c->grad;
  const float* gp[12] = {g.w1, g.b1, g.wa, g.wc, g.wp, g.bp, g.ln_w, g.ln_b, g.wkv, g.wq, g.wo, g.bo};
  for (int i = 0; i < 12; ++i)
    MHIMX_CHECK_ARG(gp[i] >= c->g && gp[i] < c->g + c->n_train, "window: every gradient view lies inside the flat gradient buffer g[0, n_train)");
  MHIMX_CHECK_ARG(g.w1 == c->g && (c->E * c->D) % 4 == 0, "window: feature.0.weight's gradient is the FIRST block of the flat gradient buffer");
  for (int i = 1; i < 12; ++i) MHIMX_CHECK_ARG(gp[i] >= c->g + c->E * c->D, "window: gradient views overlap feature.0.weight's");
  return 0;
}

}
}

extern "C" int mhimx_window_layout_of(const mhimx_step_cfg* cfg, int32_t n_bags, int64_t N, const mhimx_step_counts* cnt, mhimx_window_layout* out) {
  MHIMX_CHECK_ARG(out, "window_layout: null output");
  if (int r = check_window(cfg, n_bags, N, cnt)) return r;
  StepBufs b;
  layout(cfg, N, cnt, &b, n_bags);
  out->total = b.total; out->bag0 = b.bag0; out->bag_stride = b.bag_stride; out->grad_slab = b.gslab;
  out->bag = mhimx_step_layout{b.total, b.logits, b.losses, cfg->attn2score ? b.pscore : b.attn, b.rows_all, b.H_t, b.Hbuf, b.dact, b.z_t, b.z_s, b.g_z, b.dH};
  return 0;
}

extern "C" int mhimx_window_run(void* stream, const mhimx_step_cfg* cfg, int32_t n_bags, const float* const* X, int64_t ldx, int64_t N,
                                const int64_t* const* labels_dev, const mhimx_step_counts* cnt, const mhimx_step_seeds* seeds, int64_t host_step, void* ws,
                                int64_t ws_bytes, int32_t update) {
  if (int r = check_window(cfg, n_bags, N, cnt)) return r;
  MHIMX_CHECK_ARG(X && labels_dev && seeds && ws && ldx >= cfg->D && ldx % 4 == 0 && N * ldx * 4 < ((int64_t)1 << 32),
                  "window: null bags / labels / seeds / workspace, or a row pitch the weight-gradient product does not take");
  for (int32_t i = 0; i < n_bags; ++i) MHIMX_CHECK_ARG(X[i] && aligned16(X[i]) && labels_dev[i], "window: bag %d / its label null or not 16-byte aligned", i);
  MHIMX_CHECK_ARG(!update || (cfg->p && cfg->m && cfg->v), "window: update needs the flat optimiser buffers");
  StepBufs b;
  layout(cfg, N, cnt, &b, n_bags);
  MHIMX_CHECK_ARG(ws_bytes >= b.total && (reinterpret_cast<uintptr_t>(ws) & 255) == 0, "window: workspace too small (%lld < %lld) or not 256-byte aligned",
                  (long long)ws_bytes, (long long)b.total);
  const mhimx_step_cfg& c = *cfg;
  const mhimx_step_params &S = c.student, &T = c.teacher;
  const int64_t D = c.D, E = c.E, A = c.A, C = c.C, k = c.k, I = 512;
  const int64_t R = cnt->R, Lk = cnt->Lk, len_keep = cnt->len_keep;
  const hipStream_t st = (hipStream_t)stream;
  Carve cv(ws);
  const int64_t BS = b.bag_stride;
  auto bag = [&](int64_t off, int i) { return cv.at<char>(off) + (int64_t)i * BS; };
  float* w1p_t = cv.at<float>(b.w1p_t);
  float* wa_frag_t = cv.at<float>(b.wa_frag_t);
  float* w1p_s = cv.at<float>(b.w1p_s);
  float* wa_frag_s = cv.at<float>(b.wa_frag_s);
  float* wa_t = cv.at<float>(b.wa_t);
  float* wa_t_frag = cv.at<float>(b.wa_t_frag);
  float* wo_t = cv.at<float>(b.wo_t);
// ... 128 lines not shown
      if (int r = mhimx_abmil_pool_bwd(stream, &sc_b, &io_s, &pg)) return r;
    }
    if (int r = mhimx_merge_bwd(stream, &mwb, Hbuf, R, dH + N * E, dH, &mg, merge_ws, b.merge_ws_bytes)) return r;
    if (b.fuse_img) {
      if (int r = dpre_merge_rows(stream, dH, cv.at<char>(b.dact), rows_all, R, E, cv.at<char>(b.img), b.P0, gs(c.grad.b1), cv.at<float>(b.ws_b), b.ws_b_bytes, &lst))
        return r;
    } else if (int r = mhimx_rows_dpre_image(stream, dH, cv.at<char>(b.dact), rows_all, len_keep, E, cv.at<char>(b.img), gs(c.grad.b1), 0, cv.at<char>(b.ws_b),
                                             b.ws_b_bytes, &lst))
      return r;
    if (int r = mhimx_reduce_flush(stream, &lst)) return r;
  }

  mhimx_reduce_list lst_w;
  memset(&lst_w, 0, sizeof(lst_w));
  {
    mhimx_bag_wgrad_args ga[MHIMX_WINDOW_MAX];
    for (int i = 0; i < n_bags; ++i) {
      mhimx_bag_wgrad_args g = {};
      g.img = bag(b.img, i); g.X = X[i]; g.ldx = ldx; g.n_bag_rows = N; g.rows = reinterpret_cast<const int64_t*>(bag(b.fuse_img ? b.rows_img : b.rows_all, i));
      g.L = b.L_img; g.E = E; g.D = D;
      g.C = c.grad.w1; g.ldc = D; g.accumulate = 0; g.ws = cv.at<float>(b.wg_ws); g.ws_floats = b.wg_ws_floats; g.defer = &lst_w;
      ga[i] = g;
    }
    if (int r = mhimx_bag_wgrad_multi(stream, ga, n_bags)) return r;
  }
  {
    QChainW cw;
    const double mm = (double)c.merge_mm;
    cw.wq = (float)pow(mm, (double)n_bags);
    for (int i = 0; i < MHIMX_WINDOW_MAX; ++i) cw.w[i] = i < n_bags ? (float)((1.0 - mm) * pow(mm, (double)(n_bags - 1 - i))) : 0.f;
    SlabGaps gaps = {};
    {
      struct View { int64_t off, len; };
      const mhimx_step_grads& gr = c.grad;
      View v[11] = {{gr.b1 - c.g, E}, {gr.wa - c.g, A * E}, {gr.wc - c.g, A}, {gr.wp - c.g, C * E}, {gr.bp - c.g, C}, {gr.ln_w - c.g, E}, {gr.ln_b - c.g, E},
                    {gr.wkv - c.g, 2 * I * E}, {gr.wq - c.g, I * E}, {gr.wo - c.g, E * I}, {gr.bo - c.g, E}};
      for (int i = 1; i < 11; ++i)
        for (int j = i; j > 0 && v[j].off < v[j - 1].off; --j) { const View t = v[j]; v[j] = v[j - 1]; v[j - 1] = t; }
      int64_t at = g_lo;
      for (int i = 0; i <= 11; ++i) {
        const int64_t nxt = i < 11 ? v[i].off : c.n_train;
        if (nxt > at) { gaps.off[gaps.n] = at; gaps.len[gaps.n] = nxt - at; ++gaps.n; }
        if (i < 11 && v[i].off + v[i].len > at) at = v[i].off + v[i].len;
      }
    }
    hipLaunchKernelGGL(window_q_chain_kernel, dim3((unsigned)cdiv(k * E, 256)), dim3(256), 0, st, S.q, Hbuf + N * E, BS / 4, (int)n_bags, k * E, cw, slab0, BS / 4,
                       gaps);
    MHIMX_LAUNCH_CHECK();
  }
  if (!update) {
    if (int r = mhimx_reduce_flush(stream, &lst_w)) return r;
    hipLaunchKernelGGL(window_sum_slabs_kernel, dim3((unsigned)(cdiv(c.n_train - g_lo, 256) < 2048 ? cdiv(c.n_train - g_lo, 256) : 2048)), dim3(256), 0, st,
                       c.g + g_lo, slab0 + g_lo, BS / 4, (int)n_bags, c.n_train - g_lo);
    MHIMX_LAUNCH_CHECK();
    return 0;
  }
  mhimx_optim_args o = {};
  o.p = c.p; o.g = c.g; o.m = c.m; o.v = c.v; o.teacher = c.p_teacher; o.n_train = c.n_train; o.n_all = c.n_all; o.step = host_step; o.step_dev = c.opt_step;
  o.lr = c.lr; o.lr_table = c.lr_table; o.lr_len = c.lr_len; o.beta1 = c.beta1; o.beta2 = c.beta2; o.eps = c.eps; o.weight_decay = c.weight_decay;
  o.grad_scale = 1.f; o.ema_mm = c.ema_mm; o.mm_table = c.mm_table; o.mm_len = c.mm_len; o.zero_grad = 1; o.fold = &lst_w;
  o.g_extra = slab0; o.n_extra = n_bags; o.extra_pitch = BS / 4; o.extra_lo = g_lo; o.extra_only = 1;
  return mhimx_optim_step(stream, &o);
}

extern "C" int mhimx_step_project_ms(float* ms_out, float* empty_ms_out, int32_t cap) {
  MHIMX_CHECK_ARG(ms_out && cap >= 0, "step_project_ms: null output");
  int dev = 0;
  MHIMX_HIP(hipGetDevice(&dev));
  MHIMX_CHECK_ARG(dev >= 0 && dev < 64, "step_project_ms: device index %d", dev);
  const int n = g_proj_times.n[dev] < cap ? g_proj_times.n[dev] : cap;
  for (int i = 0; i < n; ++i) {
    MHIMX_HIP(hipEventSynchronize(g_proj_times.e[dev][i][2]));
    MHIMX_HIP(hipEventElapsedTime(ms_out + i, g_proj_times.e[dev][i][0], g_proj_times.e[dev][i][1]));
    if (empty_ms_out) MHIMX_HIP(hipEventElapsedTime(empty_ms_out + i, g_proj_times.e[dev][i][1], g_proj_times.e[dev][i][2]));
  }
  g_proj_times.n[dev] = 0;
  return n;
}

extern "C" int mhimx_step_run_many(void* stream, const mhimx_step_cfg* cfg, int32_t n_bags, const float* const* X, const int64_t* ldx, const int64_t* N,
                                   const int64_t* const* labels_dev, const mhimx_step_counts* cnt, const mhimx_step_seeds* seeds, int64_t host_step0,
                                   void* ws, int64_t ws_bytes) {
  MHIMX_CHECK_ARG(n_bags >= 1 && X && ldx && N && labels_dev && cnt && seeds, "step_run_many: null arguments");
  for (int32_t i = 0; i < n_bags; ++i)
    if (int r = mhimx_step_run(stream, cfg, X[i], ldx[i], N[i], labels_dev[i], cnt + i, seeds + i, host_step0 + i, ws, ws_bytes, 1)) return r;
  return 0;
}

namespace mhimx {
namespace {

struct PureBufs {
  int64_t w1p, wa_frag, wa_t, wa_t_frag;
  int64_t H, dact, s, stats, z, pool_ws, pool_ws_bytes;
  int64_t logits, losses, g_z;
  int64_t dH, img, ws_b, ws_b_bytes, wg_ws, wg_ws_floats;
  int64_t total;
};

int check_pure_cfg(const mhimx_step_cfg* c, int64_t N) {
  MHIMX_CHECK_ARG(c, "pure_step: null configuration");
  MHIMX_CHECK_ARG(c->E == 512 && c->A == 128 && c->C >= 1 && c->C <= 4 && c->D > 0 && c->D % 256 == 0,
                  "pure_step: shapes outside the single-pass ABMIL step (E = 512, A = 128, C <= 4, D %% 256 == 0)");
  MHIMX_CHECK_ARG(N >= 64 && N <= MHIMX_STEP_MAX_ROWS, "pure_step: row count outside 64 <= N <= %d", MHIMX_STEP_MAX_ROWS);
  const mhimx_step_params& s = c->student;
  MHIMX_CHECK_ARG(s.w1 && s.b1 && s.wa && s.wc && s.wp && s.bp, "pure_step: null student parameter");
  const mhimx_step_grads& g = c->grad;
  MHIMX_CHECK_ARG(g.w1 && g.b1 && g.wa && g.wc && g.wp && g.bp, "pure_step: null gradient view");
  MHIMX_CHECK_ARG(c->tick, "pure_step: the device dropout counter (tick) is required");
  return 0;
}

void pure_layout(const mhimx_step_cfg* c, int64_t N, PureBufs* b) {
  const int64_t D = c->D, E = c->E, A = c->A, F = sizeof(float);
  Carve cv(nullptr);
  b->w1p = cv.take_off(E * D * F);
  b->wa_frag = cv.take_off(A * E * F);
  b->wa_t = cv.take_off(E * A * F);
  b->wa_t_frag = cv.take_off(E * A * F);
  b->H = cv.take_off(N * E * F);
  b->dact = cv.take_off(N * E * 2);
  b->s = cv.take_off(N * F);
  b->stats = cv.take_off(2 * F);
  b->z = cv.take_off(E * F);
  b->pool_ws_bytes = mhimx_abmil_pool_ws_bytes(N, E, A, 0);
  b->pool_ws = cv.take_off(b->pool_ws_bytes);
  b->logits = cv.take_off(16 * F);
  b->losses = cv.take_off(4 * F);
  b->g_z = cv.take_off(E * F);
  b->dH = cv.take_off(N * E * F);
  b->img = cv.take_off(mhimx_wgrad_image_bytes(N, E));
  b->ws_b_bytes = (N + 31) / 32 * E * F;
  b->ws_b = cv.take_off(b->ws_b_bytes);
  b->wg_ws_floats = mhimx_wgrad_ws_floats(N, E, D);
  b->wg_ws = cv.take_off(b->wg_ws_floats * F);
  b->total = cv.off;
}

}
}

extern "C" int mhimx_pure_step_layout_of(const mhimx_step_cfg* cfg, int64_t N, mhimx_step_layout* out) {
  MHIMX_CHECK_ARG(out, "pure_step_layout: null output");
  if (int r = check_pure_cfg(cfg, N)) return r;
  PureBufs b;
  pure_layout(cfg, N, &b);
  *out = mhimx_step_layout{b.total, b.logits, b.losses, -1, -1, -1, b.H, b.dact, -1, b.z, b.g_z, b.dH};
  return 0;
}

extern "C" int mhimx_pure_step_run(void* stream, const mhimx_step_cfg* cfg, const float* X, int64_t ldx, int64_t N, const int64_t* label_dev,
                                   uint64_t drop_seed, int64_t host_step, void* ws, int64_t ws_bytes, int32_t update) {
  if (int r = check_pure_cfg(cfg, N)) return r;
  MHIMX_CHECK_ARG(X && label_dev && ws && ldx >= cfg->D && ldx % 4 == 0 && N * ldx * 4 < ((int64_t)1 << 32) && aligned16(X),
                  "pure_step: null bag / label / workspace, or a row pitch the weight-gradient product does not take");
  MHIMX_CHECK_ARG(!update || (cfg->p && cfg->g && cfg->m && cfg->v && cfg->n_train > 0 && cfg->n_all >= cfg->n_train),
                  "pure_step: update needs the flat optimiser buffers");
  PureBufs b;
  pure_layout(cfg, N, &b);
  MHIMX_CHECK_ARG(ws_bytes >= b.total && (reinterpret_cast<uintptr_t>(ws) & 255) == 0, "pure_step: workspace too small (%lld < %lld) or not 256-byte aligned",
                  (long long)ws_bytes, (long long)b.total);
  const mhimx_step_cfg& c = *cfg;
  const mhimx_step_params& S = c.student;
  const int64_t D = c.D, E = c.E, A = c.A, C = c.C;
  Carve cv(ws);
  float* w1p = cv.at<float>(b.w1p);
  float* wa_frag = cv.at<float>(b.wa_frag);
  float* wa_t = cv.at<float>(b.wa_t);
// ... 72 lines not shown
```

mhim_mil_amd/engine.py:

```python
from __future__ import annotations

from typing import Optional

import os

import torch

from . import mhim as mh
from . import ops
from .mhim import MHIM, BagPlan


class CommonMIL:

    def __init__(self, args=None, fused=None, graph_cache=0) -> None:
        self.training = True
        self.fused = fused
        self.graph_cache = int(graph_cache)

    def _native_step(self, tr, bag, label, n_iter, extra):
        if self.graph_cache > 0 and not extra:
            out = tr.shape_cached("forward_backward", bag, label, i=n_iter, cache=self.graph_cache)
            if out is not None:
                return out
# ... 154 lines not shown
    if chain is not None and chain.tokens is not None:
        torch.mul(chain.tokens.reshape(-1), chain.w, out=grad[chain.off:chain.off + chain.n])


def finish_tail(grad, student, n_train, scale, chain=None):
    if chain is not None and chain.tokens is not None:
        q0 = student[chain.off:chain.off + chain.n].clone()
        student[n_train:].copy_(grad[n_train:] * scale)
        torch.add(grad[chain.off:chain.off + chain.n], q0, alpha=chain.decay, out=student[chain.off:chain.off + chain.n])
        chain.tokens = None
    else:
        student[n_train:].copy_(grad[n_train:] * scale)
    grad[n_train:].zero_()


_STEP_IMAGES = os.environ.get("MHIMX_STEP_IMAGES", "1") != "0"
_WINDOW_BATCHED = os.environ.get("MHIMX_WINDOW_BATCHED", "1") != "0"
_WINDOW_WGRAD = os.environ.get("MHIMX_WINDOW_WGRAD", "0") != "0"
_WINDOW_PROJECT = os.environ.get("MHIMX_WINDOW_PROJECT", "0") != "0"


class _SplitStep:

    def __init__(self, trainer, g_fb, g_up):
        self.tr, self.g_fb, self.g_up = trainer, g_fb, g_up

    def replay(self):
        tr = self.tr
        self.g_fb.replay()
        tr._all_reduce(tr.flat.grad)
        self.g_up.replay()
        ops.step_images(None)


class FusedTrainer:

    def __init__(self, student: MHIM, teacher: Optional[MHIM], lr=2e-4, weight_decay=1e-5, betas=(0.9, 0.999), eps=1e-8,
                 mm=0.9997, main_alpha=1.0, aux_alpha=0.5, accumulation_steps=1, process_group=None, model="mhim", mm_sche=None,
                 clip_grad=None, lr_sche=None):
        if model not in ("mhim", "mhim_pure"):
            raise mh.L.MhimxError(f"FusedTrainer: model={model!r} (the path knows 'mhim' and 'mhim_pure')")
        if model == "mhim" and teacher is None:
            raise mh.L.MhimxError("FusedTrainer(model='mhim') needs the EMA teacher (modules/__init__.py:176-214 builds it)")
        if model == "mhim" and not student.merge_enable:
            raise mh.L.MhimxError("FusedTrainer(model='mhim') needs merge_enable=True: the reference's MHIM.forward rejects the Identity "
                                  "merge (mhim.py:82,351)")
        self.s, self.t = student, teacher
        self.flat = FlatState(student, teacher, step_merges=(model == "mhim"))
        self.lr, self.wd, self.betas, self.eps, self.mm = lr, weight_decay, betas, eps, mm
        self.main_alpha, self.aux_alpha = main_alpha, aux_alpha
        self.accum = max(1, int(accumulation_steps))
        self.pg = process_group
        self.comm = None
        self.world = torch.distributed.get_world_size(process_group) if self._dist() else 1
        self.model_kind = model
        self._chain, self._chain_tokens, self._q_scratch = None, None, None
        if (self.world > 1 and self.accum == 1 and model == "mhim" and student.merge_enable and student.baseline == "attn"
                and "merge.global_q_mm" in self.flat.offsets):
            rank = torch.distributed.get_rank(process_group)
            self._chain = QueryChain(self.flat.offsets["merge.global_q_mm"], student.merge.global_q_mm.numel(), float(student.merge.g_q_mm),
                                     self.world, rank)
        self._micro = 0
        self.last = {}
        dev = self.flat.student.device
        self.tick = torch.zeros(1, dtype=torch.int64, device=dev)
        self.opt_step = torch.zeros(1, dtype=torch.int64, device=dev)
        self._defer = ops.ReduceList()
        self.overlap_comm = True
        self._work_a = None
        self._capturing = False
        fo = self.flat.offsets
        self._split = fo["feature.0.bias"] + (student.feature[0].bias.numel() + 3) // 4 * 4 if "feature.0.bias" in fo else 0
        if not (self.flat.names[:2] == ["feature.0.weight", "feature.0.bias"]):
            self._split = 0
        student._tick = self.tick
        if teacher is not None:
            teacher._tick = self.tick
        self.mm_table = None if mm_sche is None else torch.as_tensor(mm_sche, dtype=torch.float32).to(dev).contiguous()
        self.clip_grad = None if clip_grad is None else float(clip_grad)
        self.lr_table = None if lr_sche is None else torch.as_tensor(lr_sche, dtype=torch.float32).to(dev).contiguous()
        self._clip_ws = torch.empty(1024, device=dev) if self.clip_grad else None
        self._g_extra = None
        self._fold_now, self._fold_list = False, None
        self._graph_pool = None
        self._cap_stream = None
        self._side = None
        self.step_dag = os.environ.get("MHIMX_STEP_DAG", "0") != "0"
        self.use_executor = os.environ.get("MHIMX_STEP_EXEC", "1") != "0"
        self._exec = None
        self.exec_max_rows = 262144
        self.single_pass = True
        self.window_streams = 4
        self.window_batched = _WINDOW_BATCHED
        self._rows_cache = {}
        self.pure_window_row_cap = 262144
        self.ragged_window_row_cap = 262144

    def _dist(self):
        return torch.distributed.is_available() and torch.distributed.is_initialized()

    def forward_backward(self, bag, label, perm=None, ids_shuffle=None, i=None):
        s, t, fl = self.s, self.t, self.flat
        x = s._check_x(bag)
        if self._nat_ok(x, i):
            if self._exec_ok(x, i, perm, ids_shuffle):
                return self._exec_step(x, label, i)
            return self._forward_backward_nat(x, label, perm, ids_shuffle, i)
        prep_s = prep_t = None
        jobs = [(ops.PREP_TICK, None, self.tick)]
        if self._micro == 0:
            jobs.append((ops.PREP_TICK, None, self.opt_step))
        if s.baseline == "attn":
            if self.model_kind == "mhim":
                jt, prep_t = t.prep_jobs(backward=False)
                jobs += jt
            js, prep_s = s.prep_jobs(backward=True)
            jobs += js
        if s.baseline == "selfattn" and _STEP_IMAGES and x.shape[0] >= 2048:
            table = {}
            for model, backward in ((t if self.model_kind == "mhim" else None, False), (s, True)):
                if model is None:
                    continue
                for layer in (model.online_encoder.layer1, model.online_encoder.layer2):
                    for w in (layer.attn.to_qkv.weight.data, layer.attn.to_out[0].weight.data):
                        img = torch.empty_like(w)
                        jobs.append((ops.PREP_PAIR, w, img))
                        table[(w.data_ptr(), False)] = img
                        if backward:
                            img_t = torch.empty((w.shape[1], w.shape[0]), device=w.device)
                            jobs.append((ops.PREP_PAIR_T, w, img_t))
                            table[(w.data_ptr(), True)] = img_t
            ops.step_images(table)
        xp = None
        if s.baseline == "attn" and s._pairable(x):
            xp = torch.empty_like(x)
            jobs.append((ops.PREP_PAIR, x, xp))
        ops.prep_batch(jobs)
        ps = x.shape[0]
        first = self._micro == 0
        gv = fl.grad_views
        if self.model_kind == "mhim":
            pre, seed_s = None, None
            if (self.single_pass and s.baseline in ("selfattn", "dsmil") and s.single_projection_ok(x) and t.single_projection_ok(x)
                    and s.act == t.act):
                tok_t = None
                if s.baseline == "selfattn":
                    tok_t = torch.empty((1 + x.shape[0], t.feature[0].weight.shape[0]), device=x.device)
                heads = [ops.ProjHead(ops.pair_planes(t.feature[0].weight.data), t.feature[0].bias.data,
                                      drop_p=t.dropout_p if t.training else 0.0, drop_seed=t._next_seed(teacher=True),
                                      out=None if tok_t is None else tok_t[1:]),
                         None]
                seed_s = s._next_seed()
                heads[1] = ops.ProjHead(ops.pair_planes(s.feature[0].weight.data), s.feature[0].bias.data, drop_p=s.dropout_p,
                                        drop_seed=seed_s, want_dact=True)
                ops.bag_project(x, heads, act=mh.L.act_code(s.act, mh._FEATURE_ACTS), drop_tick=self.tick)
                pre = (heads[1].out, heads[1].dact)
                teacher_feat, score = t.forward_teacher(x, H=heads[0].out, tok_full=tok_t)
            else:
                teacher_feat, score = t.forward_teacher(x, xp=xp, w1p=None if prep_t is None else prep_t["w1p"],
                                                        wa_frag=None if prep_t is None else prep_t.get("wa_frag"))
            mf = s.baseline == "attn"
            rows, len_keep, Lk, R = s.student_rows(ps, i, score, perm=perm, ids_shuffle=ids_shuffle, merge_first=mf)
            plan = BagPlan(rows=rows, L=len_keep, Lk=Lk, R=R, drop_seed=s._next_seed() if seed_s is None else seed_s,
                           mca_seed=s._next_seed(), training=True, merge_first=mf)
            plan.pre = pre
            if self._chain is not None:
# ... 348 lines not shown
            E=s.mlp_dim, A=s.online_encoder.attention.attention[0].weight.shape[0], C=s.n_classes, max_rows=self.exec_max_rows,
            row_cap=min(self.ragged_window_row_cap, mh.L.RAGGED_WINDOW_MAX_ROWS), max_bags=mh.L.RAGGED_WINDOW_MAX, elem=xs[0].element_size())

    def _exec_ragged_window(self, xs, labels, i, update):
        L = mh.L
        s, t, fl = self.s, self.t, self.flat
        n = len(xs)
        ex = self._exec_cfg()
        table = (L.RaggedWindowBag * n)()
        for j, (x, l) in enumerate(zip(xs, labels)):
            k_top, n_sel, len_keep, Lk, R = s.v2_counts(x.shape[0], i)
            table[j].X, table[j].ldx, table[j].N, table[j].label_dev = x.data_ptr(), x.stride(0), x.shape[0], l.data_ptr()
            table[j].cnt = L.StepCounts(k_top=k_top, n_sel=n_sel, len_keep=len_keep, Lk=Lk, R=R)
        lay = ops.ragged_window(ex["cfg"], table, n, layout_only=True)
        dev = xs[0].device
        if torch.cuda.is_current_stream_capturing():
            ws = torch.empty(lay.total, dtype=torch.uint8, device=dev)
        else:
            ws = ex.get("ws_rw")
            if ws is None or ws.numel() < lay.total or ws.device != dev:
                ws = ex["ws_rw"] = torch.full((int(lay.total * 1.25),), 255, dtype=torch.uint8, device=dev)
        for j in range(n):
            table[j].seeds = L.StepSeeds(drop_teacher=t._next_seed(teacher=True), drop_student=s._next_seed(), select=s._next_seed(),
                                         mca=s._next_seed())
        inside = bool(update and not self.clip_grad)
        ops.ragged_window(ex["cfg"], table, n, fl.step + int(inside), ws, inside, x_dtype=ops.x_dtype_of(xs))
        km, E, Cc = s.merge.k, s.mlp_dim, s.n_classes

        def view(off, cnt_, dtype=torch.float32):
            return ws[off:off + cnt_ * dtype.itemsize].view(dtype)

        lg, ls = view(lay.logits, n * 16).view(n, 16), view(lay.losses, n * 4).view(n, 4)
        Hs, Ht = view(lay.H_student, lay.rows * E).view(lay.rows, E), view(lay.H_teacher, lay.rows * E).view(lay.rows, E)
        dact = view(lay.dact, lay.rows * E, torch.float16).view(lay.rows, E)
        score, rows_all = view(lay.score, lay.rows), view(lay.rows_all, lay.rows, torch.int64)
        zt, zs = view(lay.z_teacher, n * E).view(n, E), view(lay.z_student, n * E).view(n, E)
        per = []
        for j, x in enumerate(xs):
            r0, N, cnt = int(lay.row0[j]), x.shape[0], table[j].cnt
            per.append({"logits": lg[j, :Cc], "losses": ls[j, :3], "patch_num": N, "keep_num": cnt.Lk + km, "rows": rows_all[r0:r0 + cnt.len_keep],
                        "score": score[r0:r0 + N], "R": cnt.R, "tokens": Hs[r0 + N:r0 + N + km], "H_student": Hs[r0:r0 + N],
                        "H_teacher": Ht[r0:r0 + N], "dact": dact[r0:r0 + N], "z_teacher": zt[j], "z_student": zs[j], "row0": r0})
        logits, losses = [p_["logits"] for p_ in per], [p_["losses"] for p_ in per]
        self.last = dict(per[-1], logits=logits, losses=losses, bags=per, layout=lay, table=table, ws=ws, exec="mhimx_ragged_window_run",
                         x_dtype=xs[0].dtype)
        self._micro = n
        if inside:
            fl.step += 1
            ops.step_images(None)
            self._micro = 0
        elif update:
            self.update()
        return logits, losses

    def _exec_plan(self, ex, N, i):
        import ctypes as C
        L = mh.L
        if self.model_kind == "mhim_pure":
            ent = ex["layouts"].get(("pure", N))
            if ent is None:
                lay = L.StepLayout()
                L.check(L.lib().mhimx_pure_step_layout_of(C.byref(ex["cfg"]), N, C.byref(lay)), "mhimx_pure_step_layout_of")
                ent = ex["layouts"][("pure", N)] = (None, lay)
            return ent
        k, n_sel, len_keep, Lk, R = self.s.v2_counts(N, i)
        key = (N, k, n_sel, Lk)
        ent = ex["layouts"].get(key)
        if ent is None:
            cnt = L.StepCounts(k_top=k, n_sel=n_sel, len_keep=len_keep, Lk=Lk, R=R)
            lay = L.StepLayout()
            L.check(L.lib().mhimx_step_layout_of(C.byref(ex["cfg"]), N, C.byref(cnt), C.byref(lay)), "mhimx_step_layout_of")
            ent = ex["layouts"][key] = (cnt, lay)
        return ent

    def _exec_step(self, x, label, i):
        import ctypes as C
        L = mh.L
        s, t, fl = self.s, self.t, self.flat
        if not (torch.is_tensor(label) and label.is_cuda and label.dtype == torch.int64 and label.is_contiguous() and label.device == x.device):
            raise L.MhimxError(f"label: expected a contiguous int64 tensor on the bag's device ({x.device})")
        ex = self._exec_cfg()
        N = x.shape[0]
        cnt, lay = self._exec_plan(ex, N, i)
        if torch.cuda.is_current_stream_capturing():
            ws = torch.empty(lay.total, dtype=torch.uint8, device=x.device)
        else:
            ws = ex["ws"]
            if ws is None or ws.numel() < lay.total or ws.device != x.device:
                ws = ex["ws"] = torch.full((int(lay.total * 1.25),), 255, dtype=torch.uint8, device=x.device)

        def view(off, n, dtype=torch.float32):
            return ws[off:off + n * dtype.itemsize].view(dtype)

        if self.model_kind == "mhim_pure":
            seed = s._next_seed()
            update = bool(self._fold_now)
            L.check(L.lib().mhimx_pure_step_run(ops._stream(), C.byref(ex["cfg"]), x.data_ptr(), x.stride(0), N, label.data_ptr(), seed,
                                                fl.step + int(update), ws.data_ptr(), ws.numel(), int(update)), "mhimx_pure_step_run")
            if update:
                fl.step += 1
            logits, losses = view(lay.logits, s.n_classes), view(lay.losses, 3)
            self.last = {"logits": logits, "losses": losses, "patch_num": N, "keep_num": N, "rows": None, "score": None, "R": 0, "tokens": None,
                         "H_student": view(lay.H_student, N * s.mlp_dim).view(N, s.mlp_dim), "H_teacher": None, "ws": ws, "exec": True}
            if update:
                ops.step_images(None)
                self._micro = 0
            else:
                self._micro += 1
            return logits, losses
        seeds = L.StepSeeds(drop_teacher=t._next_seed(teacher=True), drop_student=s._next_seed(), select=s._next_seed(), mca=s._next_seed())
        update = bool(self._fold_now)
        L.check(L.lib().mhimx_step_run(ops._stream(), C.byref(ex["cfg"]), x.data_ptr(), x.stride(0), N, label.data_ptr(), C.byref(cnt), C.byref(seeds),
                                       fl.step + int(update), ws.data_ptr(), ws.numel(), int(update)), "mhimx_step_run")
        if update:
            fl.step += 1
        km, E = s.merge.k, s.mlp_dim
        Hs = view(lay.H_student, (N + km) * E).view(N + km, E)
        logits, losses = view(lay.logits, s.n_classes), view(lay.losses, 3)
        rows_all = view(lay.rows_all, cnt.len_keep + km, torch.int64)
        self.last = {"logits": logits, "losses": losses, "patch_num": N, "keep_num": cnt.Lk + km, "rows": rows_all[:cnt.len_keep],
                     "score": view(lay.score, N), "R": cnt.R, "tokens": Hs[N:], "H_student": Hs[:N],
                     "H_teacher": view(lay.H_teacher, N * E).view(N, E), "ws": ws, "exec": True}
        if self._chain is not None:
            self._chain.tokens = self._chain_tokens = Hs[N:]
        if update:
            ops.step_images(None)
            self._micro = 0
        else:
            self._micro += 1
        return logits, losses

    def run_steps(self, bags, labels, i=None):
        import ctypes as C
        L = mh.L
        n = len(bags)
        if n == 0 or len(labels) != n:
            raise L.MhimxError(f"run_steps: {n} bags, {len(labels)} labels")
        its = list(i) if isinstance(i, (list, tuple)) else [None if i is None else i + j for j in range(n)]
        if len(its) != n:
            raise L.MhimxError(f"run_steps: {len(its)} iteration indices for {n} bags")
        xs = [self.s._check_x(b) for b in bags]
        if self._micro != 0:
            raise L.MhimxError("run_steps: called inside an accumulation window (a fresh update is required)")
        if self.clip_grad or self.accum != 1 or self.world != 1 or not all(self._exec_ok(x, it) and self._nat_ok(x, it) for x, it in zip(xs, its)):
            out = None
            for b, l, it in zip(bags, labels, its):
                out = self.train_step(b, l, i=it)
            return out
        for x, l in zip(xs, labels):
            if not (torch.is_tensor(l) and l.is_cuda and l.dtype == torch.int64 and l.is_contiguous() and l.device == x.device and l.numel() >= 1):
                raise L.MhimxError(f"run_steps: every label must be a contiguous int64 tensor on its bag's device ({x.device})")
        ex = self._exec_cfg()
        plans = [self._exec_plan(ex, x.shape[0], it) for x, it in zip(xs, its)]
        total = max(p[1].total for p in plans)
        ws = ex["ws"]
        if ws is None or ws.numel() < total or ws.device != xs[0].device:
            ws = ex["ws"] = torch.empty(int(total * 1.25), dtype=torch.uint8, device=xs[0].device)
        Xp = (C.c_void_p * n)(*[x.data_ptr() for x in xs])
        ld = (C.c_int64 * n)(*[x.stride(0) for x in xs])
        Ns = (C.c_int64 * n)(*[x.shape[0] for x in xs])
        lab = (C.c_void_p * n)(*[l.data_ptr() for l in labels])
        lay = plans[-1][1]
        if self.model_kind == "mhim_pure":
            drop_seeds = (C.c_uint64 * n)(*[self.s._next_seed() for _ in range(n)])
            L.check(L.lib().mhimx_pure_step_run_many(ops._stream(), C.byref(ex["cfg"]), n, Xp, ld, Ns, lab, drop_seeds, self.flat.step + 1, ws.data_ptr(),
                                                     ws.numel()), "mhimx_pure_step_run_many")
            self.flat.step += n
            ops.step_images(None)
            N, E = xs[-1].shape[0], self.s.mlp_dim
            logits, losses = ws[lay.logits:lay.logits + 4 * self.s.n_classes].view(torch.float32), ws[lay.losses:lay.losses + 12].view(torch.float32)
            self.last = {"logits": logits, "losses": losses, "patch_num": N, "keep_num": N, "rows": None, "score": None, "R": 0, "tokens": None,
                         "H_student": ws[lay.H_student:lay.H_student + N * E * 4].view(torch.float32).view(N, E), "H_teacher": None, "ws": ws,
                         "exec": True}
            return logits, losses
        cnts = (L.StepCounts * n)(*[p[0] for p in plans])
        seeds = (L.StepSeeds * n)()
        for j in range(n):
            seeds[j] = L.StepSeeds(drop_teacher=self.t._next_seed(teacher=True), drop_student=self.s._next_seed(), select=self.s._next_seed(),
                                   mca=self.s._next_seed())
        L.check(L.lib().mhimx_step_run_many(ops._stream(), C.byref(ex["cfg"]), n, Xp, ld, Ns, lab, cnts, seeds, self.flat.step + 1, ws.data_ptr(),
                                            ws.numel()), "mhimx_step_run_many")
        self.flat.step += n
        ops.step_images(None)
        return ws[lay.logits:lay.logits + 4 * self.s.n_classes].view(torch.float32), ws[lay.losses:lay.losses + 12].view(torch.float32)

    def _forward_backward_nat(self, x, label, perm, ids_shuffle, i):
        first = self._micro == 0
        for tns, nm in ((label, "label"), (perm, "perm"), (ids_shuffle, "ids_shuffle")):
            if torch.is_tensor(tns) and not (tns.is_cuda and tns.dtype == torch.int64 and tns.is_contiguous() and tns.device == x.device):
                raise mh.L.MhimxError(f"{nm}: expected a contiguous int64 tensor on the bag's device ({x.device}), got {tns.dtype} on {tns.device}")
        with ops.pinned_stream():
            res = self._nat_prep([x], i, with_opt_tick=first, split=True)
            prep_t, preps = res[0], res[1]
            preps[0]["_ride_jobs"] = res[2] if len(res) > 2 else None
            hook = self._mid_hook if (first and self.overlap_comm and self.comm is None and self.world > 1 and self.accum == 1
                                      and not self._capturing and self._split > 0) else None
# ... 336 lines not shown
            scale = sync_flat_gradient(fl.grad, fl.student, fl.n_train, self.world, self.pg, self.comm, self._chain)
        self._apply(scale)

    def _all_reduce(self, buf):
        if self.comm is not None:
            self.comm.allreduce(buf)
        else:
            torch.distributed.all_reduce(buf, group=self.pg)

    def _apply(self, scale):
        fl = self.flat
        ops.step_images(None)
        fl.step += 1
        ops.optim_step(fl.student, fl.grad, fl.m, fl.v, fl.teacher if (self.model_kind == "mhim" and not fl.same_teacher) else None, fl.n_train,
                       fl.step, lr=self.lr, beta1=self.betas[0], beta2=self.betas[1], eps=self.eps, weight_decay=self.wd,
                       grad_scale=scale, ema_mm=self.mm, zero_grad=True, step_dev=self.opt_step, mm_table=self.mm_table,
                       lr_table=self.lr_table, g_extra=self._g_extra, clip_norm=self.clip_grad, ws=self._clip_ws, fold=self._fold_list)
        self._g_extra = None
        self._fold_list = None
        self._micro = 0

    def capture(self, bag, label, warmup=2, **kw):
        assert self.accum == 1, "graph capture covers a full step (accumulation_steps == 1)"
        if self.s.mrh_sche is not None:
            raise mh.L.MhimxError("capture(): the HAM-ratio schedule (mrh_sche) changes the number of masked rows per iteration; "
                                  "run such a model with eager train_step calls, or capture one graph per schedule value")
        self._capturing = True
        try:
            return self._capture(bag, label, warmup, **kw)
        finally:
            self._capturing = False

    def _capture(self, bag, label, warmup, **kw):
        if self._cap_stream is None:
            self._cap_stream = torch.cuda.Stream()
        cs = self._cap_stream
        cs.wait_stream(torch.cuda.current_stream())
        with torch.cuda.stream(cs):
            for _ in range(warmup):
                self.train_step(bag, label, **kw)
        torch.cuda.current_stream().wait_stream(cs)
        torch.cuda.synchronize()
        if self._graph_pool is None:
            self._graph_pool = torch.cuda.graph_pool_handle()
        if self.world > 1:
            fl = self.flat
            g_fb, g_up = torch.cuda.CUDAGraph(), torch.cuda.CUDAGraph()
            with torch.cuda.graph(g_fb, pool=self._graph_pool, stream=cs, capture_error_mode="thread_local"):
                self.forward_backward(bag, label, **kw)
                fill_tail(fl.grad, fl.student, fl.n_train, self._chain)
            ops.step_images(None)
            self._all_reduce(fl.grad)
            scale = 1.0 / self.world
            with torch.cuda.graph(g_up, pool=self._graph_pool, stream=cs, capture_error_mode="thread_local"):
                finish_tail(fl.grad, fl.student, fl.n_train, scale, self._chain)
                self._apply(scale)
            fl.grad.zero_()
            return _SplitStep(self, g_fb, g_up)
        g = torch.cuda.CUDAGraph()
        with torch.cuda.graph(g, pool=self._graph_pool, stream=cs):
            self.train_step(bag, label, **kw)
        return g

    def capture_steps(self, bags, labels, warmup=1, **kw):
        assert self.accum == 1 and self.world == 1, "capture_steps: one process, one bag per update"
        if self.s.mrh_sche is not None:
            raise mh.L.MhimxError("capture_steps(): the HAM-ratio schedule changes the launch shapes per iteration")
        self._capturing = True
        try:
            if self._cap_stream is None:
                self._cap_stream = torch.cuda.Stream()
            cs = self._cap_stream
            cs.wait_stream(torch.cuda.current_stream())
            with torch.cuda.stream(cs):
                for _ in range(warmup):
                    for b, l in zip(bags, labels):
                        self.train_step(b, l, **kw)
            torch.cuda.current_stream().wait_stream(cs)
            torch.cuda.synchronize()
            if self._graph_pool is None:
                self._graph_pool = torch.cuda.graph_pool_handle()
            g = torch.cuda.CUDAGraph()
            with torch.cuda.graph(g, pool=self._graph_pool, stream=cs):
                for b, l in zip(bags, labels):
                    self.train_step(b, l, **kw)
            return g
        finally:
            self._capturing = False

    def shape_cached(self, what, bag, label, i=None, cache=64):
        x = bag[0] if bag.dim() == 3 else bag
        s, t = self.s, self.t
        if not (self.accum == 1 and self.world == 1 and x.is_cuda and x.dim() == 2 and not self._capturing and self._micro == 0):
            return None
        nat = self._nat_ok(x, i)
        auto = (not nat) and s.baseline in ("selfattn", "dsmil") and (self.model_kind != "mhim" or s.v2_counts(x.shape[0], i) is not None)
        if not (nat or auto):
            return None
        counts = s.v2_counts(x.shape[0], i) if self.model_kind == "mhim" else None
        st = getattr(self, "_shape_graphs", None)
        if st is None:
            st = self._shape_graphs = {"graphs": {}, "seen": {}, "arena": None, "bad": set()}
        key = (what, tuple(x.shape), x.dtype, x.device.index, counts, s.training, None if t is None else t.training, s.merge_enable,
               float(self.main_alpha), float(self.aux_alpha), tuple(label.shape))
        scal = None
        if what == "train_step":
            scal = (None if self.lr_table is not None else float(self.lr), tuple(self.betas), float(self.eps), float(self.wd),
                    None if self.mm_table is not None else float(self.mm))
        if key in st["bad"]:
            return None
        ent = st["graphs"].get(key)
        if ent is not None and ent[8] != scal:
            st["graphs"].pop(key)
            ent = None
            n_re = st.setdefault("rescaled", {})
            n_re[key] = n_re.get(key, 0) + 1
            if n_re[key] > 2:
                st["bad"].add(key)
                st["seen"].pop(key, None)
                return None
            st["seen"][key] = 2
        if len(st["seen"]) > 4096:
            st["seen"] = {k_: v_ for k_, v_ in st["seen"].items() if k_ in st["graphs"]}
        fn = self.train_step if what == "train_step" else self.forward_backward
        if auto and self._cap_stream is None:
            self._cap_stream = torch.cuda.Stream()
        if ent is None:
            st["seen"][key] = st["seen"].get(key, 0) + 1
            if st["seen"][key] < (3 if auto else 2):
                if auto:
                    cur = torch.cuda.current_stream()
                    self._cap_stream.wait_stream(cur)
                    with torch.cuda.stream(self._cap_stream):
                        logits, losses = fn(bag, label, i=i)
                    cur.wait_stream(self._cap_stream)
                else:
                    logits, losses = fn(bag, label, i=i)
                return logits, losses, self.last["patch_num"], self.last["keep_num"]
            while len(st["graphs"]) >= max(1, int(cache)):
                st["graphs"].pop(next(iter(st["graphs"])))
            need = x.numel()
            ar = st["arena"]
            if ar is None or ar.numel() < need or ar.dtype != x.dtype or ar.device != x.device:
                ar = st["arena"] = torch.empty(need, dtype=x.dtype, device=x.device)
            xs, ls = ar[:need].view(x.shape), torch.empty_like(label)
            if self._cap_stream is None:
                self._cap_stream = torch.cuda.Stream()
            if self._graph_pool is None:
                self._graph_pool = torch.cuda.graph_pool_handle()
            cs = self._cap_stream
            cs.wait_stream(torch.cuda.current_stream())
            torch.cuda.synchronize()
            g = torch.cuda.CUDAGraph()
            micro, host_step = self._micro, self.flat.step
            self._capturing = True
            try:
                with torch.cuda.graph(g, pool=self._graph_pool, stream=cs):
                    logits, losses = fn(xs, ls, i=i)
            except Exception as exc:
                if isinstance(exc, mh.L.MhimxError):
                    self._capturing = False
                    self._micro, self.flat.step = micro, host_step
                    self._fold_list = None
                    self._defer = ops.ReduceList()
                    ops.step_images(None)
                    raise
                st["bad"].add(key)
                st.setdefault("errors", []).append(repr(exc))
                self._micro, self.flat.step = micro, host_step
                self._fold_list = None
                self._defer = ops.ReduceList()
# ... 32 lines not shown
```

Baseline: 33.68 million patch-instances/s.

## Carry bf16x3 weight images from Adam/EMA into the next chained bag step

Adds a carry variant of the Adam+EMA kernel that writes the updated student w1, teacher w1 and teacher scorer weights straight into the split-bf16 (hi/lo) and fragment-layout images the next step's GEMMs consume. Consecutive bags in a captured graph, and in step_run_many, are chained so the next step skips the early prep/convert jobs and only runs the tick and row riders. The intent is to cut the separate weight-image conversion passes and their launches between steps. The cost is extra stores in the optimizer kernel and strict alignment and eligibility checks, with a fallback to the unchained path.

```diff
diff --git a/include/mhimx.h b/include/mhimx.h
--- a/include/mhimx.h
+++ b/include/mhimx.h
@@ -363,6 +363,12 @@
 } mhimx_optim_args;
 int mhimx_optim_step(void* stream, const mhimx_optim_args* a);
 
+#define MHIMX_CARRY_MAX 4
+typedef struct { int32_t kind; int64_t off, R, C; float* student; float* teacher; } mhimx_carry_entry;
+typedef struct { mhimx_carry_entry e[MHIMX_CARRY_MAX]; int32_t n; uint64_t* tick; } mhimx_optim_carry;
+int mhimx_optim_step_carry(void* stream, const mhimx_optim_args* a, const mhimx_optim_carry* carry);
+int64_t mhimx_prep_image_offset(int32_t kind, int64_t R, int64_t C, int64_t idx);
+
 #define MHIMX_STEP_MAX_ROWS 262144
 #define MHIMX_WINDOW_MAX 8
 typedef struct {
@@ -414,6 +420,11 @@
 int mhimx_step_run_many(void* stream, const mhimx_step_cfg* cfg, int32_t n_bags, const float* const* X, const int64_t* ldx, const int64_t* N,
                         const int64_t* const* labels_dev, const mhimx_step_counts* cnt, const mhimx_step_seeds* seeds, int64_t host_step0,
                         void* ws, int64_t ws_bytes);
+#define MHIMX_CHAIN_IN 1
+#define MHIMX_CHAIN_OUT 2
+int mhimx_step_run_chain(void* stream, const mhimx_step_cfg* cfg, const float* X, int64_t ldx, int64_t N, const int64_t* label_dev,
+                         const mhimx_step_counts* cnt, const mhimx_step_seeds* seeds, int64_t host_step, void* ws, int64_t ws_bytes, int32_t update,
+                         int32_t chain);
 
 int mhimx_pure_step_layout_of(const mhimx_step_cfg* cfg, int64_t N, mhimx_step_layout* out);
 int mhimx_pure_step_run(void* stream, const mhimx_step_cfg* cfg, const float* X, int64_t ldx, int64_t N, const int64_t* label_dev,
diff --git a/mhim_mil_amd/_lib.py b/mhim_mil_amd/_lib.py
--- a/mhim_mil_amd/_lib.py
+++ b/mhim_mil_amd/_lib.py
@@ -164,6 +164,18 @@
                 ("ema_mm", C.c_float), ("mm_table", C.c_void_p), ("mm_len", C.c_int64), ("zero_grad", C.c_int32),
                 ("g_extra", C.c_void_p), ("n_extra", C.c_int64), ("extra_pitch", C.c_int64), ("clip_norm", C.c_float),
                 ("ws", C.c_void_p), ("ws_floats", C.c_int64), ("fold", C.c_void_p), ("extra_lo", C.c_int64), ("extra_only", C.c_int32)]
+
+
+CARRY_MAX = 4
+CHAIN_IN, CHAIN_OUT = 1, 2
+
+
+class CarryEntry(C.Structure):
+    _fields_ = [("kind", C.c_int32), ("off", C.c_int64), ("R", C.c_int64), ("C", C.c_int64), ("student", C.c_void_p), ("teacher", C.c_void_p)]
+
+
+class OptimCarry(C.Structure):
+    _fields_ = [("e", CarryEntry * CARRY_MAX), ("n", C.c_int32), ("tick", C.c_void_p)]
 
 
 class StepParams(C.Structure):
@@ -316,6 +328,8 @@
     "mhimx_adam_ema": (C.c_int, [_P, _P, _P, _P, _P, _P, _I64, _I64, _I64, _F, _F, _F, _F, _F, _F, _F, _I32, _P, _P, _I64]),
     "mhimx_bmm_chain": (C.c_int, [_P, C.POINTER(BmmStep), _I32, _I32, _P]),
     "mhimx_optim_step": (C.c_int, [_P, C.POINTER(OptimArgs)]),
+    "mhimx_optim_step_carry": (C.c_int, [_P, C.POINTER(OptimArgs), C.POINTER(OptimCarry)]),
+    "mhimx_prep_image_offset": (_I64, [_I32, _I64, _I64, _I64]),
     "mhimx_stream_copy": (C.c_int, [_P, _P, _P, _I64]),
     "mhimx_tick": (C.c_int, [_P, _P]),
     "mhimx_layernorm_fwd": (C.c_int, [_P, _P, _I64, _I64, _P, _P, _P, _P, _P]),
@@ -360,6 +374,7 @@
     "mhimx_step_counts_of": (C.c_int, [_I64, C.c_double, C.c_double, C.c_double, C.POINTER(StepCounts)]),
     "mhimx_step_layout_of": (C.c_int, [C.POINTER(StepCfg), _I64, C.POINTER(StepCounts), C.POINTER(StepLayout)]),
     "mhimx_step_run": (C.c_int, [_P, C.POINTER(StepCfg), _P, _I64, _I64, _P, C.POINTER(StepCounts), C.POINTER(StepSeeds), _I64, _P, _I64, _I32]),
+    "mhimx_step_run_chain": (C.c_int, [_P, C.POINTER(StepCfg), _P, _I64, _I64, _P, C.POINTER(StepCounts), C.POINTER(StepSeeds), _I64, _P, _I64, _I32, _I32]),
     "mhimx_step_project_ms": (C.c_int, [_P, _P, _I32]),
     "mhimx_window_layout_of": (C.c_int, [C.POINTER(StepCfg), _I32, _I64, C.POINTER(StepCounts), C.POINTER(WindowLayout)]),
     "mhimx_window_run": (C.c_int, [_P, C.POINTER(StepCfg), _I32, _P, _I64, _I64, _P, C.POINTER(StepCounts), C.POINTER(StepSeeds), _I64, _P, _I64, _I32]),
diff --git a/mhim_mil_amd/csrc/adam_ema_body.hpp b/mhim_mil_amd/csrc/adam_ema_body.hpp
--- /dev/null
+++ b/mhim_mil_amd/csrc/adam_ema_body.hpp
@@ -0,0 +1,116 @@
+  __shared__ float sc[4];
+  __shared__ float clip_red[256];
+  if (ex.clip_norm > 0.f) {
+    float a = 0.f;
+    for (int i = threadIdx.x; i < ex.n_parts; i += 256) a += ex.sq_parts[i];
+    clip_red[threadIdx.x] = a;
+    __syncthreads();
+    for (int o = 128; o > 0; o >>= 1) {
+      if ((int)threadIdx.x < o) clip_red[threadIdx.x] += clip_red[threadIdx.x + o];
+      __syncthreads();
+    }
+  }
+  if (threadIdx.x == 0) {
+    int64_t step = step_host;
+    if (step_dev) step = (int64_t)step_dev[0];
+    if (ex.lr_table) {
+      int64_t i = step - 1;
+      i = i < 0 ? 0 : (i >= ex.lr_len ? ex.lr_len - 1 : i);
+      lr = ex.lr_table[i];
+    }
+    if (step_dev || ex.lr_table) {
+      const double t = (double)step;
+      lr_over_bc1 = (float)((double)lr / (1.0 - exp(t * ln_beta1)));
+      bc2s = (float)sqrt(1.0 - exp(t * ln_beta2));
+    }
+    float coef = 1.f;
+    if (ex.clip_norm > 0.f) {
+      coef = ex.clip_norm / (sqrtf(clip_red[0]) + 1e-6f);
+      coef = coef > 1.f ? 1.f : coef;
+    }
+    sc[3] = coef;
+    if (mm_table) {
+      int64_t i = step - 1;
+      i = i < 0 ? 0 : (i >= mm_len ? mm_len - 1 : i);
+      mm = mm_table[i];
+    }
+    sc[0] = lr_over_bc1; sc[1] = bc2s; sc[2] = mm;
+  }
+  __syncthreads();
+  lr_over_bc1 = sc[0];
+  bc2s = sc[1];
+  mm = sc[2];
+  gscale *= sc[3];
+  const int64_t n4 = n_all / 4;
+  const bool vec_ok = ((reinterpret_cast<uintptr_t>(p) | reinterpret_cast<uintptr_t>(g) | reinterpret_cast<uintptr_t>(m) |
+                        reinterpret_cast<uintptr_t>(v) | reinterpret_cast<uintptr_t>(teacher)) & 15) == 0;
+  for (int64_t q = (int64_t)blockIdx.x * blockDim.x + threadIdx.x; q * 4 < n_all; q += (int64_t)gridDim.x * blockDim.x) {
+    const int64_t i0 = q * 4;
+    if (vec_ok && q < n4 && (i0 + 4 <= n_train || i0 >= n_train)) {
+      float4 w = reinterpret_cast<float4*>(p)[q];
+      int64_t cpos = -1;
+      int cf = 0;
+      if constexpr (CARRY) {
+        for (int f = 0; f < ctp->count; ++f)
+          if (i0 >= ctp->off[f] && i0 < ctp->off[f] + ctp->n[f]) { cf = f; cpos = carry_pos(*ctp, f, i0 - ctp->off[f]); }
+      }
+      if (i0 < n_train) {
+        const bool slabs = i0 >= ex.extra_lo;
+        bool g_skip = false;
+        if constexpr (CARRY) {
+          for (int f = 0; f < ex.fold.count; ++f)
+            if (i0 >= ex.fold.off[f] && i0 < ex.fold.off[f] + ex.fold.n[f] && !ex.fold.accumulate[f]) g_skip = true;
+        }
+        float4 gi = ((slabs && ex.extra_only) || g_skip) ? make_float4(0.f, 0.f, 0.f, 0.f) : reinterpret_cast<float4*>(g)[q];
+        float4 mi = reinterpret_cast<float4*>(m)[q], vi = reinterpret_cast<float4*>(v)[q];
+        for (int f = 0; f < ex.fold.count; ++f)
+          if (i0 >= ex.fold.off[f] && i0 < ex.fold.off[f] + ex.fold.n[f]) {
+            const float4 sv = fold_sum4(ex.fold.parts[f], ex.fold.n[f], i0 - ex.fold.off[f], ex.fold.G[f]);
+            if (ex.fold.accumulate[f]) { gi.x += sv.x; gi.y += sv.y; gi.z += sv.z; gi.w += sv.w; }
+            else gi = sv;
+          }
+        for (int64_t z = 0; slabs && z < ex.n_extra; ++z) {
+          const float4 e = *reinterpret_cast<const float4*>(ex.g_extra + z * ex.extra_pitch + i0);
+          gi.x += e.x; gi.y += e.y; gi.z += e.z; gi.w += e.w;
+        }
+        adam_one(w.x, gi.x, mi.x, vi.x, lr_over_bc1, bc2s, beta1, beta2, eps, wd, gscale);
+        adam_one(w.y, gi.y, mi.y, vi.y, lr_over_bc1, bc2s, beta1, beta2, eps, wd, gscale);
+        adam_one(w.z, gi.z, mi.z, vi.z, lr_over_bc1, bc2s, beta1, beta2, eps, wd, gscale);
+        adam_one(w.w, gi.w, mi.w, vi.w, lr_over_bc1, bc2s, beta1, beta2, eps, wd, gscale);
+        reinterpret_cast<float4*>(m)[q] = mi;
+        reinterpret_cast<float4*>(v)[q] = vi;
+        reinterpret_cast<float4*>(p)[q] = w;
+        if (zero_grad) reinterpret_cast<float4*>(g)[q] = make_float4(0.f, 0.f, 0.f, 0.f);
+        if constexpr (CARRY) {
+          if (cpos >= 0 && ctp->s[cf]) carry_store4(ctp->s[cf] + cpos, w);
+        }
+      }
+      if (teacher) {
+        float4 t = reinterpret_cast<float4*>(teacher)[q];
+        t.x = t.x * mm + w.x * (1.f - mm); t.y = t.y * mm + w.y * (1.f - mm);
+        t.z = t.z * mm + w.z * (1.f - mm); t.w = t.w * mm + w.w * (1.f - mm);
+        reinterpret_cast<float4*>(teacher)[q] = t;
+        if constexpr (CARRY) {
+          if (cpos >= 0 && ctp->t[cf]) carry_store4(ctp->t[cf] + cpos, t);
+        }
+      }
+      continue;
+    }
+    for (int64_t i = i0; i < i0 + 4 && i < n_all; ++i) {
+      float w = p[i];
+      if (i < n_train) {
+        const bool slabs = i >= ex.extra_lo;
+        float gi = (slabs && ex.extra_only) ? 0.f : g[i], mi = m[i], vi = v[i];
+        for (int64_t z = 0; slabs && z < ex.n_extra; ++z) gi += ex.g_extra[z * ex.extra_pitch + i];
+        adam_one(w, gi, mi, vi, lr_over_bc1, bc2s, beta1, beta2, eps, wd, gscale);
+        m[i] = mi;
+        v[i] = vi;
+        p[i] = w;
+        if (zero_grad) g[i] = 0.f;
+      }
+      if (teacher) teacher[i] = teacher[i] * mm + w * (1.f - mm);
+    }
+  }
+  if constexpr (CARRY) {
+    if (ctp->tick && blockIdx.x == 0 && threadIdx.x == 0) ctp->tick[0] += 1;
+  }
diff --git a/mhim_mil_amd/csrc/optim.hip b/mhim_mil_amd/csrc/optim.hip
--- a/mhim_mil_amd/csrc/optim.hip
+++ b/mhim_mil_amd/csrc/optim.hip
@@ -336,107 +336,47 @@
   w = w - lr_over_bc1 * (mi / (sqrtf(vi) / bc2s + eps));
 }
 
+struct CarryTab { int kind[MHIMX_CARRY_MAX]; int64_t off[MHIMX_CARRY_MAX], n[MHIMX_CARRY_MAX]; uint32_t C[MHIMX_CARRY_MAX];
+                  __bf16* s[MHIMX_CARRY_MAX]; __bf16* t[MHIMX_CARRY_MAX]; int count; uint64_t* tick; };
+typedef __bf16 carry_b4 __attribute__((ext_vector_type(4)));
+MHIMX_DEV void carry_store4(__bf16* img, const float4& x) {
+  const float xs[4] = {x.x, x.y, x.z, x.w};
+  carry_b4 hi, lo;
+#pragma unroll
+  for (int i = 0; i < 4; ++i) {
+    const __bf16 h = (__bf16)xs[i];
+    hi[i] = h;
+    lo[i] = (__bf16)(xs[i] - (float)h);
+  }
+  *reinterpret_cast<carry_b4*>(img) = hi;
+  *reinterpret_cast<carry_b4*>(img + 8) = lo;
+}
+MHIMX_DEV int64_t carry_pos(const CarryTab& ct, int f, int64_t rel) {
+  int64_t unit = rel >> 3;
+  if (ct.kind[f] == 4) {
+    const uint32_t C = ct.C[f], r = (uint32_t)rel / C, c = (uint32_t)rel - r * C;
+    unit = ((int64_t)(r >> 5) * (C >> 4) + (c >> 4)) * 64 + (r & 31) + 32 * ((c >> 3) & 1);
+  }
+  return unit * 16 + (rel & 4);
+}
+
 __global__ __launch_bounds__(256) void adam_ema_kernel(
     float* __restrict__ p, float* __restrict__ g, float* __restrict__ m, float* __restrict__ v, float* __restrict__ teacher,
     int64_t n_train, int64_t n_all, float lr_over_bc1, float bc2s, float beta1, float beta2, float eps, float wd, float gscale,
     float mm, int zero_grad, const uint64_t* __restrict__ step_dev, float lr, const float* __restrict__ mm_table, int64_t mm_len,
     int64_t step_host, double ln_beta1, double ln_beta2, OptimExtra ex) {
-  __shared__ float sc[4];
-  __shared__ float clip_red[256];
-  if (ex.clip_norm > 0.f) {
-    float a = 0.f;
-    for (int i = threadIdx.x; i < ex.n_parts; i += 256) a += ex.sq_parts[i];
-    clip_red[threadIdx.x] = a;
-    __syncthreads();
-    for (int o = 128; o > 0; o >>= 1) {
-      if ((int)threadIdx.x < o) clip_red[threadIdx.x] += clip_red[threadIdx.x + o];
-      __syncthreads();
-    }
-  }
-  if (threadIdx.x == 0) {
-    int64_t step = step_host;
-    if (step_dev) step = (int64_t)step_dev[0];
-    if (ex.lr_table) {
-      int64_t i = step - 1;
-      i = i < 0 ? 0 : (i >= ex.lr_len ? ex.lr_len - 1 : i);
-      lr = ex.lr_table[i];
-    }
-    if (step_dev || ex.lr_table) {
-      const double t = (double)step;
-      lr_over_bc1 = (float)((double)lr / (1.0 - exp(t * ln_beta1)));
-      bc2s = (float)sqrt(1.0 - exp(t * ln_beta2));
-    }
-    float coef = 1.f;
-    if (ex.clip_norm > 0.f) {
-      coef = ex.clip_norm / (sqrtf(clip_red[0]) + 1e-6f);
-      coef = coef > 1.f ? 1.f : coef;
-    }
-    sc[3] = coef;
-    if (mm_table) {
-      int64_t i = step - 1;
-      i = i < 0 ? 0 : (i >= mm_len ? mm_len - 1 : i);
-      mm = mm_table[i];
-    }
-    sc[0] = lr_over_bc1; sc[1] = bc2s; sc[2] = mm;
-  }
-  __syncthreads();
-  lr_over_bc1 = sc[0];
-  bc2s = sc[1];
-  mm = sc[2];
-  gscale *= sc[3];
-  const int64_t n4 = n_all / 4;
-  const bool vec_ok = ((reinterpret_cast<uintptr_t>(p) | reinterpret_cast<uintptr_t>(g) | reinterpret_cast<uintptr_t>(m) |
-                        reinterpret_cast<uintptr_t>(v) | reinterpret_cast<uintptr_t>(teacher)) & 15) == 0;
-  for (int64_t q = (int64_t)blockIdx.x * blockDim.x + threadIdx.x; q * 4 < n_all; q += (int64_t)gridDim.x * blockDim.x) {
-    const int64_t i0 = q * 4;
-    if (vec_ok && q < n4 && (i0 + 4 <= n_train || i0 >= n_train)) {
-      float4 w = reinterpret_cast<float4*>(p)[q];
-      if (i0 < n_train) {
-        const bool slabs = i0 >= ex.extra_lo;
-        float4 gi = (slabs && ex.extra_only) ? make_float4(0.f, 0.f, 0.f, 0.f) : reinterpret_cast<float4*>(g)[q];
-        float4 mi = reinterpret_cast<float4*>(m)[q], vi = reinterpret_cast<float4*>(v)[q];
-        for (int f = 0; f < ex.fold.count; ++f)
-          if (i0 >= ex.fold.off[f] && i0 < ex.fold.off[f] + ex.fold.n[f]) {
-            const float4 sv = fold_sum4(ex.fold.parts[f], ex.fold.n[f], i0 - ex.fold.off[f], ex.fold.G[f]);
-            if (ex.fold.accumulate[f]) { gi.x += sv.x; gi.y += sv.y; gi.z += sv.z; gi.w += sv.w; }
-            else gi = sv;
-          }
-        for (int64_t z = 0; slabs && z < ex.n_extra; ++z) {
-          const float4 e = *reinterpret_cast<const float4*>(ex.g_extra + z * ex.extra_pitch + i0);
-          gi.x += e.x; gi.y += e.y; gi.z += e.z; gi.w += e.w;
-        }
-        adam_one(w.x, gi.x, mi.x, vi.x, lr_over_bc1, bc2s, beta1, beta2, eps, wd, gscale);
-        adam_one(w.y, gi.y, mi.y, vi.y, lr_over_bc1, bc2s, beta1, beta2, eps, wd, gscale);
-        adam_one(w.z, gi.z, mi.z, vi.z, lr_over_bc1, bc2s, beta1, beta2, eps, wd, gscale);
-        adam_one(w.w, gi.w, mi.w, vi.w, lr_over_bc1, bc2s, beta1, beta2, eps, wd, gscale);
-        reinterpret_cast<float4*>(m)[q] = mi;
-        reinterpret_cast<float4*>(v)[q] = vi;
-        reinterpret_cast<float4*>(p)[q] = w;
-        if (zero_grad) reinterpret_cast<float4*>(g)[q] = make_float4(0.f, 0.f, 0.f, 0.f);
-      }
-      if (teacher) {
-        float4 t = reinterpret_cast<float4*>(teacher)[q];
-        t.x = t.x * mm + w.x * (1.f - mm); t.y = t.y * mm + w.y * (1.f - mm);
-        t.z = t.z * mm + w.z * (1.f - mm); t.w = t.w * mm + w.w * (1.f - mm);
-        reinterpret_cast<float4*>(teacher)[q] = t;
-      }
-      continue;
-    }
-    for (int64_t i = i0; i < i0 + 4 && i < n_all; ++i) {
-      float w = p[i];
-      if (i < n_train) {
-        const bool slabs = i >= ex.extra_lo;
-        float gi = (slabs && ex.extra_only) ? 0.f : g[i], mi = m[i], vi = v[i];
-        for (int64_t z = 0; slabs && z < ex.n_extra; ++z) gi += ex.g_extra[z * ex.extra_pitch + i];
-        adam_one(w, gi, mi, vi, lr_over_bc1, bc2s, beta1, beta2, eps, wd, gscale);
-        m[i] = mi;
-        v[i] = vi;
-        p[i] = w;
-        if (zero_grad) g[i] = 0.f;
-      }
-      if (teacher) teacher[i] = teacher[i] * mm + w * (1.f - mm);
-    }
-  }
+  constexpr bool CARRY = false;
+  constexpr const CarryTab* ctp = nullptr;
+#include "adam_ema_body.hpp"
+}
+__global__ __launch_bounds__(256) void adam_ema_carry_kernel(
+    float* __restrict__ p, float* __restrict__ g, float* __restrict__ m, float* __restrict__ v, float* __restrict__ teacher,
+    int64_t n_train, int64_t n_all, float lr_over_bc1, float bc2s, float beta1, float beta2, float eps, float wd, float gscale,
+    float mm, int zero_grad, const uint64_t* __restrict__ step_dev, float lr, const float* __restrict__ mm_table, int64_t mm_len,
+    int64_t step_host, double ln_beta1, double ln_beta2, OptimExtra ex, CarryTab ct) {
+  constexpr bool CARRY = true;
+  const CarryTab* ctp = &ct;
+#include "adam_ema_body.hpp"
 }
 
 }
@@ -476,7 +416,55 @@
   return 0;
 }
 
-extern "C" int mhimx_optim_step(void* stream, const mhimx_optim_args* a) {
+namespace mhimx {
+namespace {
+int carry_fill(const mhimx_optim_args* a, const mhimx_optim_carry* c, CarryTab* ct) {
+  MHIMX_CHECK_ARG(c->n >= 0 && c->n <= MHIMX_CARRY_MAX, "optim_step_carry: 0..%d entries", MHIMX_CARRY_MAX);
+  MHIMX_CHECK_ARG(!(a->clip_norm > 0.f) && a->n_extra == 0, "optim_step_carry: not with clipping or gradient slabs");
+  MHIMX_CHECK_ARG(aligned16(a->p) && aligned16(a->g) && aligned16(a->m) && aligned16(a->v) && (!a->teacher || aligned16(a->teacher)),
+                  "optim_step_carry: every flat buffer 16-byte aligned");
+  *ct = CarryTab{};
+  ct->count = c->n;
+  ct->tick = c->tick;
+  for (int i = 0; i < c->n; ++i) {
+    const mhimx_carry_entry& e = c->e[i];
+    MHIMX_CHECK_ARG(e.kind == 1 || e.kind == 4, "optim_step_carry: entry %d: image kind 1 or 4", i);
+    MHIMX_CHECK_ARG(e.R > 0 && e.C > 0 && e.C % 16 == 0 && (e.kind != 4 || e.R % 32 == 0) && e.R * e.C < ((int64_t)1 << 31),
+                    "optim_step_carry: entry %d: C %% 16 == 0 (fragment image: R %% 32 == 0), fewer than 2^31 elements", i);
+    MHIMX_CHECK_ARG(e.off >= 0 && e.off % 8 == 0 && e.off < a->n_train && e.off + e.R * e.C <= a->n_train,
+                    "optim_step_carry: entry %d: an offset that is a multiple of 8 and a range inside [0, n_train)", i);
+    MHIMX_CHECK_ARG((!e.student || aligned16(e.student)) && (!e.teacher || (aligned16(e.teacher) && a->teacher)),
+                    "optim_step_carry: entry %d: 16-byte aligned images, a teacher image needs the teacher buffer", i);
+    for (int j = 0; j < i; ++j)
+      MHIMX_CHECK_ARG(e.off + e.R * e.C <= c->e[j].off || c->e[j].off + c->e[j].R * c->e[j].C <= e.off, "optim_step_carry: entries %d and %d overlap", j, i);
+    ct->kind[i] = e.kind; ct->off[i] = e.off; ct->n[i] = e.R * e.C; ct->C[i] = (uint32_t)e.C;
+    ct->s[i] = reinterpret_cast<__bf16*>(e.student); ct->t[i] = reinterpret_cast<__bf16*>(e.teacher);
+  }
+  return 0;
+}
+}
+}
+
+static int optim_step_impl(void* stream, const mhimx_optim_args* a, const mhimx_optim_carry* carry);
+
+extern "C" int mhimx_optim_step(void* stream, const mhimx_optim_args* a) { return optim_step_impl(stream, a, nullptr); }
+extern "C" int mhimx_optim_step_carry(void* stream, const mhimx_optim_args* a, const mhimx_optim_carry* carry) {
+  MHIMX_CHECK_ARG(carry, "optim_step_carry: null carry table");
+  return optim_step_impl(stream, a, carry);
+}
+
+extern "C" int64_t mhimx_prep_image_offset(int32_t kind, int64_t R, int64_t C, int64_t idx) {
+  MHIMX_CHECK_ARG((kind == 1 || kind == 4) && R > 0 && C > 0 && C % 16 == 0 && (kind != 4 || R % 32 == 0) && idx >= 0 && idx < R * C,
+                  "prep_image_offset: kind 1 or 4, C %% 16 == 0 (kind 4: R %% 32 == 0), 0 <= idx < R C");
+  int64_t unit = idx >> 3;
+  if (kind == 4) {
+    const int64_t r = idx / C, c = idx % C;
+    unit = ((r >> 5) * (C >> 4) + (c >> 4)) * 64 + (r & 31) + 32 * ((c >> 3) & 1);
+  }
+  return unit * 16 + (idx & 7);
+}
+
+static int optim_step_impl(void* stream, const mhimx_optim_args* a, const mhimx_optim_carry* carry) {
   MHIMX_CHECK_ARG(a, "optim_step: null args");
   MHIMX_CHECK_ARG(!a->mm_table || a->mm_len > 0, "optim_step: empty momentum schedule");
   MHIMX_CHECK_ARG(!a->lr_table || a->lr_len > 0, "optim_step: empty learning-rate schedule");
@@ -487,6 +475,9 @@
   MHIMX_CHECK_ARG(a->extra_lo >= 0 && a->extra_lo % 4 == 0 && (a->n_extra > 0 || (a->extra_lo == 0 && !a->extra_only)),
                   "optim_step: extra_lo (a multiple of 4) / extra_only describe the gradient slabs of g_extra");
   int64_t step = a->step < 1 ? 1 : a->step;
+  CarryTab ct{};
+  if (carry)
+    if (int r = carry_fill(a, carry, &ct)) return r;
   if (a->n_all == 0) return 0;
   OptimExtra ex{a->lr_table, a->lr_len, a->g_extra, a->n_extra, a->extra_pitch, a->clip_norm > 0.f ? a->clip_norm : 0.f, a->ws, 0, {}, a->extra_lo, a->extra_only};
   if (a->fold) {
@@ -523,10 +514,16 @@
   const double bc1 = 1.0 - pow((double)a->beta1, (double)step);
   const double bc2 = 1.0 - pow((double)a->beta2, (double)step);
   const int64_t blocks = cdiv(a->n_all, 1024) < 2048 ? cdiv(a->n_all, 1024) : 2048;
-  hipLaunchKernelGGL(adam_ema_kernel, dim3((unsigned)blocks), dim3(256), 0, (hipStream_t)stream, a->p, a->g, a->m, a->v,
-                     a->teacher, a->n_train, a->n_all, (float)((double)a->lr / bc1), (float)sqrt(bc2), a->beta1, a->beta2, a->eps, a->weight_decay,
-                     a->grad_scale, a->ema_mm, a->zero_grad, a->step_dev, a->lr, a->mm_table, a->mm_len, step, log((double)a->beta1),
-                     log((double)a->beta2), ex);
+  if (carry)
+    hipLaunchKernelGGL(adam_ema_carry_kernel, dim3((unsigned)blocks), dim3(256), 0, (hipStream_t)stream, a->p, a->g, a->m, a->v,
+                       a->teacher, a->n_train, a->n_all, (float)((double)a->lr / bc1), (float)sqrt(bc2), a->beta1, a->beta2, a->eps, a->weight_decay,
+                       a->grad_scale, a->ema_mm, a->zero_grad, a->step_dev, a->lr, a->mm_table, a->mm_len, step, log((double)a->beta1),
+                       log((double)a->beta2), ex, ct);
+  else
+    hipLaunchKernelGGL(adam_ema_kernel, dim3((unsigned)blocks), dim3(256), 0, (hipStream_t)stream, a->p, a->g, a->m, a->v,
+                       a->teacher, a->n_train, a->n_all, (float)((double)a->lr / bc1), (float)sqrt(bc2), a->beta1, a->beta2, a->eps, a->weight_decay,
+                       a->grad_scale, a->ema_mm, a->zero_grad, a->step_dev, a->lr, a->mm_table, a->mm_len, step, log((double)a->beta1),
+                       log((double)a->beta2), ex);
   MHIMX_LAUNCH_CHECK();
   return 0;
 }
diff --git a/mhim_mil_amd/csrc/step.hip b/mhim_mil_amd/csrc/step.hip
--- a/mhim_mil_amd/csrc/step.hip
+++ b/mhim_mil_amd/csrc/step.hip
@@ -208,6 +208,12 @@
 
 extern "C" int mhimx_step_run(void* stream, const mhimx_step_cfg* cfg, const float* X, int64_t ldx, int64_t N, const int64_t* label_dev,
                               const mhimx_step_counts* cnt, const mhimx_step_seeds* seeds, int64_t host_step, void* ws, int64_t ws_bytes, int32_t update) {
+  return mhimx_step_run_chain(stream, cfg, X, ldx, N, label_dev, cnt, seeds, host_step, ws, ws_bytes, update, 0);
+}
+
+extern "C" int mhimx_step_run_chain(void* stream, const mhimx_step_cfg* cfg, const float* X, int64_t ldx, int64_t N, const int64_t* label_dev,
+                                    const mhimx_step_counts* cnt, const mhimx_step_seeds* seeds, int64_t host_step, void* ws, int64_t ws_bytes, int32_t update,
+                                    int32_t chain) {
   if (int r = check_cfg(cfg, N, cnt)) return r;
   MHIMX_CHECK_ARG(X && label_dev && seeds && ws && ldx >= cfg->D && ldx % 4 == 0 && N * ldx * 4 < ((int64_t)1 << 32) && aligned16(X),
                   "step: null bag / label / seeds / workspace, or a row pitch the weight-gradient product does not take");
@@ -238,6 +244,27 @@
   const uint64_t* tick = c.tick;
   const hipStream_t main_st = (hipStream_t)stream, side_st = (hipStream_t)c.side_stream;
   const bool dag = c.side_stream != nullptr && c.side_stream != stream;
+  const bool carry_in = (chain & MHIMX_CHAIN_IN) != 0, carry_out = (chain & MHIMX_CHAIN_OUT) != 0;
+  MHIMX_CHECK_ARG((chain & ~(MHIMX_CHAIN_IN | MHIMX_CHAIN_OUT)) == 0, "step: unknown chain bits %d", (int)chain);
+  MHIMX_CHECK_ARG(!chain || !dag, "step: the DAG form (side_stream) takes no chain bits");
+  MHIMX_CHECK_ARG(!carry_out || (update && c.p_teacher), "step: carrying the next step's preparation needs update = 1 and the EMA teacher's flat buffer");
+  mhimx_optim_carry carry = {};
+  if (chain) {
+    const int64_t F = sizeof(float);
+    MHIMX_CHECK_ARG(b.w1p_t == 0 && b.wa_frag_t == align_up(E * D * F, 256) && b.w1p_s == b.wa_frag_t + align_up(A * E * F, 256),
+                    "step: the carried images are not the first three buffers of the layout");
+  }
+  if (carry_out) {
+    const int64_t o_s = S.w1 - c.p, o_t = T.w1 - c.p_teacher, o_a = T.wa - c.p_teacher;
+    carry.e[0] = mhimx_carry_entry{1, o_s, E, D, w1p_s, o_t == o_s ? w1p_t : nullptr};
+    carry.n = 1;
+    if (o_t != o_s) carry.e[carry.n++] = mhimx_carry_entry{1, o_t, E, D, nullptr, w1p_t};
+    carry.e[carry.n++] = mhimx_carry_entry{4, o_a, A, E, nullptr, wa_frag_t};
+    carry.tick = c.tick;
+    for (int i = 0; i < carry.n; ++i)
+      MHIMX_CHECK_ARG(carry.e[i].off >= 0 && carry.e[i].off % 8 == 0 && carry.e[i].off + carry.e[i].R * carry.e[i].C <= c.n_train,
+                      "step: carry needs feature.0.weight and the teacher's scorer weight as 8-element aligned views of the flat buffers' trained part");
+  }
   hipEvent_t* ev = nullptr;
   if (dag)
     if (int r = g_dag_events.get(&ev)) return r;
@@ -246,7 +273,7 @@
   mw_prep.E = E; mw_prep.k = k; mw_prep.heads = 8; mw_prep.dim_head = 64;
   mw_prep.q_param = S.q; mw_prep.ln_w = S.ln_w; mw_prep.ln_b = S.ln_b; mw_prep.wkv = S.wkv; mw_prep.wq = S.wq; mw_prep.wo = S.wo; mw_prep.bo = S.bo;
   mw_prep.mm = c.merge_mm; mw_prep.prec = MHIMX_PREC_BF16X3; mw_prep.drop_tick = tick; mw_prep.rep = 1.f;
-  {
+  if (!carry_in) {
     mhimx_prep_job early[8];
     int n = 0;
     early[n++] = mhimx_prep_job{3, nullptr, reinterpret_cast<float*>(c.tick), 1, 1};
@@ -257,13 +284,19 @@
     early[n++] = mhimx_prep_job{10, nullptr, reinterpret_cast<float*>(rows_all + len_keep), N, k};
     if (int r = mhimx_prep_batch(stream, early, n)) return r;
   }
-  mhimx_prep_job late[6];
+  mhimx_prep_job late[8];
+  int n_late = 6;
   late[0] = mhimx_prep_job{4, S.wa, wa_frag_s, A, E};
   late[1] = mhimx_prep_job{0, S.wa, wa_t, A, E};
   late[2] = mhimx_prep_job{5, S.wa, wa_t_frag, A, E};
   late[3] = mhimx_prep_job{0, S.wo, wo_t, E, I};
   late[4] = mhimx_prep_job{2, S.q, q_old, 1, k * E};
   late[5] = mhimx_prep_job{6, reinterpret_cast<const float*>(&mw_prep), static_cast<float*>(merge_ws), R, b.merge_ws_bytes};
+  if (carry_in) {
+    if (c.opt_step) late[n_late++] = mhimx_prep_job{3, nullptr, reinterpret_cast<float*>(c.opt_step), 1, 1};
+    late[n_late++] = mhimx_prep_job{10, nullptr, reinterpret_cast<float*>(rows_all + len_keep), N, k};
+  }
+  static_assert(sizeof(late) / sizeof(late[0]) <= MHIMX_PREP_MAX, "the riders are one job table");
 
   {
     mhimx_bag_project_args a = {};
@@ -297,7 +330,7 @@
     io.ws = cv.at<char>(b.pool_ws_t); io.ws_bytes = b.pool_ws_t_bytes;
     if (c.attn2score) { io.wp = T.wp; io.C = C; io.cproj = cv.at<float>(b.cproj_t); io.bp = T.bp; io.pscore = cv.at<float>(b.pscore); }
     io.no_backward = 1;
-    io.ride_jobs = late; io.n_ride_jobs = 6;
+    io.ride_jobs = late; io.n_ride_jobs = n_late;
     if (int r = mhimx_abmil_pool_fwd(stream, &sc_t, &io)) return r;
     if (c.attn2score) score = io.pscore;
     else {
@@ -413,6 +446,7 @@
   o.p = c.p; o.g = c.g; o.m = c.m; o.v = c.v; o.teacher = c.p_teacher; o.n_train = c.n_train; o.n_all = c.n_all; o.step = host_step; o.step_dev = c.opt_step;
   o.lr = c.lr; o.lr_table = c.lr_table; o.lr_len = c.lr_len; o.beta1 = c.beta1; o.beta2 = c.beta2; o.eps = c.eps; o.weight_decay = c.weight_decay;
   o.grad_scale = 1.f; o.ema_mm = c.ema_mm; o.mm_table = c.mm_table; o.mm_len = c.mm_len; o.zero_grad = 1; o.fold = lm;
+  if (carry_out) return mhimx_optim_step_carry(stream, &o, &carry);
   return mhimx_optim_step(stream, &o);
 }
 
@@ -707,8 +741,17 @@
                                    const int64_t* const* labels_dev, const mhimx_step_counts* cnt, const mhimx_step_seeds* seeds, int64_t host_step0,
                                    void* ws, int64_t ws_bytes) {
   MHIMX_CHECK_ARG(n_bags >= 1 && X && ldx && N && labels_dev && cnt && seeds, "step_run_many: null arguments");
-  for (int32_t i = 0; i < n_bags; ++i)
-    if (int r = mhimx_step_run(stream, cfg, X[i], ldx[i], N[i], labels_dev[i], cnt + i, seeds + i, host_step0 + i, ws, ws_bytes, 1)) return r;
+  bool chained = cfg && cfg->p && cfg->p_teacher && !(cfg->side_stream && cfg->side_stream != stream) && aligned16(cfg->p) && aligned16(cfg->g) &&
+                 aligned16(cfg->m) && aligned16(cfg->v) && aligned16(cfg->p_teacher);
+  if (chained) {
+    auto view_ok = [&](const float* w, const float* base, int64_t n) { return w && w >= base && (w - base) % 8 == 0 && (w - base) + n <= cfg->n_train; };
+    chained = view_ok(cfg->student.w1, cfg->p, cfg->E * cfg->D) && view_ok(cfg->teacher.w1, cfg->p_teacher, cfg->E * cfg->D) &&
+              view_ok(cfg->teacher.wa, cfg->p_teacher, cfg->A * cfg->E);
+  }
+  for (int32_t i = 0; i < n_bags; ++i) {
+    const int32_t chain = chained ? ((i > 0 ? MHIMX_CHAIN_IN : 0) | (i + 1 < n_bags ? MHIMX_CHAIN_OUT : 0)) : 0;
+    if (int r = mhimx_step_run_chain(stream, cfg, X[i], ldx[i], N[i], labels_dev[i], cnt + i, seeds + i, host_step0 + i, ws, ws_bytes, 1, chain)) return r;
+  }
   return 0;
 }
 
diff --git a/mhim_mil_amd/engine.py b/mhim_mil_amd/engine.py
--- a/mhim_mil_amd/engine.py
+++ b/mhim_mil_amd/engine.py
@@ -260,6 +260,7 @@
         self._clip_ws = torch.empty(1024, device=dev) if self.clip_grad else None
         self._g_extra = None
         self._fold_now, self._fold_list = False, None
+        self._chain_link = None
         self._graph_pool = None
         self._cap_stream = None
         self._side = None
@@ -774,7 +775,12 @@
         ex = self._exec_cfg()
         N = x.shape[0]
         cnt, lay = self._exec_plan(ex, N, i)
-        if torch.cuda.is_current_stream_capturing():
+        link = self._chain_link
+        if link is not None:
+            ws = link["ws"]
+            if ws is None:
+                ws = link["ws"] = torch.empty(link["total"], dtype=torch.uint8, device=x.device)
+        elif torch.cuda.is_current_stream_capturing():
             ws = torch.empty(lay.total, dtype=torch.uint8, device=x.device)
         else:
             ws = ex["ws"]
@@ -802,8 +808,16 @@
             return logits, losses
         seeds = L.StepSeeds(drop_teacher=t._next_seed(teacher=True), drop_student=s._next_seed(), select=s._next_seed(), mca=s._next_seed())
         update = bool(self._fold_now)
-        L.check(L.lib().mhimx_step_run(ops._stream(), C.byref(ex["cfg"]), x.data_ptr(), x.stride(0), N, label.data_ptr(), C.byref(cnt), C.byref(seeds),
-                                       fl.step + int(update), ws.data_ptr(), ws.numel(), int(update)), "mhimx_step_run")
+        if link is not None:
+            j, n = link["j"], link["n"]
+            bits = (L.CHAIN_IN if j > 0 else 0) | (L.CHAIN_OUT if j + 1 < n else 0)
+            L.check(L.lib().mhimx_step_run_chain(ops._stream(), C.byref(ex["cfg"]), x.data_ptr(), x.stride(0), N, label.data_ptr(), C.byref(cnt),
+                                                 C.byref(seeds), fl.step + int(update), ws.data_ptr(), ws.numel(), int(update), bits),
+                    "mhimx_step_run_chain")
+            link["j"] = j + 1
+        else:
+            L.check(L.lib().mhimx_step_run(ops._stream(), C.byref(ex["cfg"]), x.data_ptr(), x.stride(0), N, label.data_ptr(), C.byref(cnt),
+                                           C.byref(seeds), fl.step + int(update), ws.data_ptr(), ws.numel(), int(update)), "mhimx_step_run")
         if update:
             fl.step += 1
         km, E = s.merge.k, s.mlp_dim
@@ -1306,11 +1320,31 @@
                 self._graph_pool = torch.cuda.graph_pool_handle()
             g = torch.cuda.CUDAGraph()
             with torch.cuda.graph(g, pool=self._graph_pool, stream=cs):
+                self._chain_link = self._chain_plan(bags, kw)
                 for b, l in zip(bags, labels):
                     self.train_step(b, l, **kw)
             return g
         finally:
+            self._chain_link = None
             self._capturing = False
+
+    def _chain_plan(self, bags, kw):
+        n = len(bags)
+        if (n < 2 or self.model_kind != "mhim" or self.clip_grad or self.accum != 1 or self.world != 1 or self.step_dag or self.flat.same_teacher
+                or kw.get("perm") is not None or kw.get("ids_shuffle") is not None or isinstance(kw.get("i"), (list, tuple))):
+            return None
+        i = kw.get("i")
+        xs = [self.s._check_x(b) for b in bags]
+        if not all(self._exec_ok(x, i) and self._nat_ok(x, i) for x in xs):
+            return None
+        ex = self._exec_cfg()
+        cfg, fl = ex["cfg"], self.flat
+        for w, base, n_el in ((cfg.student.w1, fl.student.data_ptr(), cfg.E * cfg.D), (cfg.teacher.w1, fl.teacher.data_ptr(), cfg.E * cfg.D),
+                              (cfg.teacher.wa, fl.teacher.data_ptr(), cfg.A * cfg.E)):
+            if w < base or (w - base) % 32 or (w - base) // 4 + n_el > fl.n_train or base % 16:
+                return None
+        total = max(self._exec_plan(ex, x.shape[0], i)[1].total for x in xs)
+        return {"j": 0, "n": n, "total": int(total), "ws": None}
 
     def shape_cached(self, what, bag, label, i=None, cache=64):
         x = bag[0] if bag.dim() == 3 else bag
```

Result: no change. 33.53 million patch-instances/s (-0.5%).
